# vadimkantorov/convasr

Measured on AMD Instinct MI355X. Metric: audio-seconds/sec/node (fwd+bwd+CTC) at bs64x15s, higher is better.
Workload: dtype bf16

## Files before the change

convasr_amd/_lib.py:

```python
import ctypes
import os

import torch

_HERE = os.path.dirname(os.path.abspath(__file__))
LIB_PATH = os.environ.get('CONVASR_HIP_LIB') or os.path.join(_HERE, 'libconvasr_hip.so')

F32, BF16, I16, F16 = 0, 1, 2, 3
LOSS_SCALER_FLOATS = 8
ACT_NONE, ACT_RELU, ACT_HARDTANH, ACT_LEAKY_RELU = 0, 1, 2, 3
PACK_FWD, PACK_DGRAD = 0, 1
W_REFERENCE, W_KMAJOR = 0, 1
METRIC_CHARS, METRIC_WORDS = 0, 1
METRIC_MAX_LEN = 16383

c_int, c_i64, c_u64, c_f32, c_p = ctypes.c_int, ctypes.c_int64, ctypes.c_uint64, ctypes.c_float, ctypes.c_void_p

_SIGNATURES = dict(
	convasr_abi_version = (c_int, []),
	convasr_last_error = (ctypes.c_char_p, []),
	convasr_convert_layout = (c_int, [c_p, c_int, c_i64, c_i64, c_i64, c_p, c_int, c_i64, c_i64, c_i64, c_int, c_int, c_int, c_p]),
	convasr_signal_absmax = (c_int, [c_p, c_int, c_int, c_int, c_p, c_p]),
	convasr_logmel_fwd = (c_int, [c_p, c_int, c_p, c_p, c_p, c_int, c_p, c_p, c_p, c_int, c_int, c_int, c_int, c_int, c_f32, c_p]),
	convasr_instnorm_fwd = (c_int, [c_p, c_int, c_i64, c_i64, c_i64, c_p, c_int, c_i64, c_i64, c_i64, c_p, c_int, c_int, c_int, c_int, c_f32, c_p]),
	convasr_instnorm_running_fwd = (c_int, [c_p, c_int, c_i64, c_i64, c_i64, c_p, c_int, c_i64, c_i64, c_i64, c_int, c_int, c_int, c_int, c_f32, c_p, c_p, c_p, c_f32, c_int, c_p, c_p]),
	convasr_output_lengths = (c_int, [c_p, c_int, c_int, c_p, c_p]),
	convasr_conv_cout_pad = (c_int, [c_int]),
	convasr_pack_conv_weight = (c_int, [c_p, c_p, c_p, c_int, c_int, c_int, c_int, c_int, c_p]),
	convasr_fold2_geometry = (c_int, [c_int, c_int, ctypes.POINTER(c_int), ctypes.POINTER(c_int)]),
	convasr_fold2_pack_weight = (c_int, [c_p, c_int, c_p, c_int, c_int, c_int, c_int, c_int, c_p]),
	convasr_fold2_unfold_wgrad = (c_int, [c_p, c_p, c_int, c_int, c_int, c_int, c_int, c_int, c_p]),
	convasr_conv1d_fwd = (c_int, [c_p, c_p, c_p, c_int, c_int, c_int, c_int, c_int, c_int, c_int, c_int, c_int, c_int, c_int, c_p, c_p, c_p, c_p, c_int, c_f32, c_f32, c_p, c_p, c_p]),
	convasr_conv_stats_max_rows = (c_int, [c_int, c_int]),
	convasr_grouped_conv1d_fwd = (c_int, [c_p, c_p, c_i64, c_i64, c_i64, c_p, c_p, c_int, c_int, c_int, c_int, c_int, c_int, c_int, c_int, c_int, c_int, c_int, c_p]),
	convasr_grouped_conv1d_dgrad = (c_int, [c_p, c_p, c_p, c_i64, c_i64, c_i64, c_p, c_int, c_int, c_int, c_int, c_int, c_int, c_int, c_int, c_int, c_int, c_p]),
	convasr_grouped_conv1d_wgrad_workspace_bytes = (c_i64, [c_int, c_int, c_int, c_int, c_int]),
	convasr_grouped_conv1d_wgrad = (c_int, [c_p, c_p, c_p, c_p, c_i64, c_i64, c_i64, c_p, c_p, c_int, c_int, c_int, c_int, c_int, c_int, c_int, c_int, c_int, c_int, c_int, c_p]),
	convasr_reduce_rows = (c_int, [c_p, c_int, c_int, c_p, c_p]),
	convasr_debug_set_conv_v2 = (c_int, [c_int]),
	convasr_conv1d_wgrad_workspace_bytes = (c_i64, [c_int, c_int, c_int, c_int, c_int, c_int, c_int, c_int]),
	convasr_conv1d_wgrad = (c_int, [c_p, c_p, c_p, c_p, c_p, c_int, c_int, c_int, c_int, c_int, c_int, c_int, c_int, c_int, c_int, c_int, c_int, c_p]),
	convasr_bn_finalize = (c_int, [c_p, c_int, c_i64, c_p, c_p, c_p, c_p, c_f32, c_f32, c_p, c_p, c_p, c_p, c_int, c_p, c_p]),
	convasr_bn_eval_scale_shift = (c_int, [c_p, c_p, c_p, c_p, c_f32, c_p, c_p, c_int, c_p]),
	convasr_bn_act_fwd = (c_int, [c_p, c_p, c_int, c_p, c_p, c_int, c_p, c_p, c_p, c_int, c_f32, c_f32, c_f32, c_u64, c_u64, c_p, c_p, c_int, c_int, c_int, c_p, c_p]),
	convasr_bn_bwd_workspace_bytes = (c_i64, [c_int, c_int, c_int]),
	convasr_bn_act_bwd_reduce = (c_int, [c_p, c_p, c_p, c_int, c_p, c_p, c_p, c_p, c_int, c_p, c_p, c_p, c_p, c_p, c_p, c_int, c_f32, c_f32, c_f32, c_u64, c_u64, c_p, c_p, c_p, c_p, c_p, c_p, c_p, c_p, c_int, c_int, c_int, c_int, c_p, c_p]),
	convasr_bn_act_bwd_apply = (c_int, [c_p, c_p, c_p, c_int, c_p, c_int, c_p, c_p, c_int, c_f32, c_f32, c_f32, c_u64, c_u64, c_p, c_p, c_int, c_int, c_int, c_p, c_p]),
	convasr_bn_bwd_apply = (c_int, [c_p, c_p, c_p, c_int, c_p, c_p, c_p, c_p, c_p, c_p, c_int, c_int, c_int, c_int, c_p]),
	convasr_log_softmax_fwd = (c_int, [c_p, c_p, c_i64, c_int, c_p]),
	convasr_log_softmax_bwd = (c_int, [c_p, c_p, c_p, c_i64, c_int, c_p]),
	convasr_ctc_workspace_bytes = (c_i64, [c_int, c_int, c_int]),
	convasr_ctc_loss = (c_int, [c_p, c_p, c_p, c_p, c_p, c_p, c_p, c_int, c_int, c_int, c_int, c_int, c_p]),
	convasr_ctc_loss_supported = (c_int, [c_int, c_int, c_int, c_int]),
	convasr_ctc_loss_long_states_per_block = (c_int, []),
	convasr_ctc_loss_long_chunk_frames = (c_int, []),
	convasr_ctc_loss_long_workspace_bytes = (c_i64, [c_int, c_int, c_int, c_int]),
	convasr_ctc_loss_long = (c_int, [c_p, c_p, c_p, c_p, c_p, c_p, c_p, c_i64, c_int, c_int, c_int, c_int, c_int, c_int, c_p]),
	convasr_scale_rows = (c_int, [c_p, c_p, c_p, c_i64, c_p, c_int, c_i64, c_p]),
	convasr_loss_head = (c_int, [c_p, c_p, c_i64, c_p, c_int, c_f32, c_p, c_p, c_p, c_p, c_f32, c_p]),
	convasr_entropy = (c_int, [c_p, c_p, c_p, c_int, c_int, c_int, c_f32, c_p]),
	convasr_weighted_mean_entropy = (c_int, [c_p, c_p, c_p, c_int, c_int, c_int, c_int, c_f32, c_p]),
	convasr_argmax = (c_int, [c_p, c_p, c_i64, c_int, c_p]),
	convasr_sumsq_workspace_bytes = (c_i64, []),
	convasr_sumsq = (c_int, [c_p, c_i64, c_p, c_p, c_p, c_f32, c_p, c_p]),
	convasr_sgd_step = (c_int, [c_p, c_p, c_p, c_p, c_i64, c_p, c_f32, c_f32, c_f32, c_f32, c_int, c_int, c_p, c_f32, c_p, c_int, c_p, c_p, c_p, c_p]),
	convasr_adamw_step = (c_int, [c_p, c_p, c_p, c_p, c_i64, c_p, c_f32, c_f32, c_f32, c_f32, c_f32, c_f32, c_p, c_p, c_p, c_f32, c_p, c_int, c_p, c_p, c_p, c_p]),
	convasr_conv1d_dgrad_bn_reduce = (c_int, [c_p, c_p, c_p, c_int, c_int, c_int, c_int, c_int, c_int, c_int, c_int, c_int, c_p, c_p, c_p, c_p, c_p, c_int, c_f32, c_f32, c_f32, c_u64, c_u64, c_p, c_p, c_p, c_p, c_p, c_p]),
	convasr_bn_bwd_finalize = (c_int, [c_p, c_int, c_p, c_p, c_p, c_p, c_p, c_p, c_int, c_i64, c_int, c_p]),
	convasr_novograd_step = (c_int, [c_p, c_p, c_p, c_p, c_p, c_p, c_p, c_int, c_i64, c_p, c_int, c_p, c_p, c_f32, c_f32, c_f32, c_f32, c_f32, c_f32, c_int, c_int, c_p, c_p, c_f32, c_p, c_int, c_p, c_p, c_p, c_p]),
	convasr_step_begin = (c_int, [c_p, c_p]),
	convasr_conv1x1_grouped = (c_int, [c_int, c_p, c_p, c_p, c_p, c_p, c_p, c_p, c_p, c_int, c_int, c_int, ctypes.POINTER(c_int), c_p]),
	convasr_add16 = (c_int, [c_p, c_p, c_p, c_i64, c_int, c_p]),
	convasr_bn_bwd_reduce_many_workspace_bytes = (c_i64, [c_int, c_int, c_int, c_int]),
	convasr_bn_bwd_reduce_many = (c_int, [c_p, c_p, c_f32, c_p, c_int, c_p, c_p, c_p, c_p, c_p, c_p, c_p, c_p, c_p, c_int, c_int, c_int, c_int, c_p]),
	convasr_pack_dgrad_item_bytes = (c_int, []),
	convasr_pack_dgrad_grouped = (c_int, [c_p, c_int, c_int, c_p]),
	convasr_bn_finalize_grouped = (c_int, [c_int, c_p, c_int, c_i64, c_p, c_p, c_p, c_p, c_p, c_p, c_p, c_p, c_int, c_p]),
	convasr_bn_bwd_finalize_grouped = (c_int, [c_int, c_p, c_p, c_p, c_p, c_p, c_p, c_p, c_p, c_p, c_i64, c_int, c_p]),
	convasr_bn_bwd_apply_grouped = (c_int, [c_p, c_int, c_p, c_p, c_p, c_int, c_int, c_int, c_int, c_p]),
	convasr_wgrad1x1_grouped_workspace_bytes = (c_i64, [c_int, c_p, c_p, c_int, c_int]),
	convasr_wgrad1x1_grouped = (c_int, [c_int, c_p, c_p, c_p, c_p, c_p, c_p, c_p, c_p, c_int, c_int, c_int, c_p]),
	convasr_copy = (c_int, [c_p, c_p, c_i64, c_p]),
	convasr_colsum_workspace_bytes = (c_i64, [c_i64, c_int]),
	convasr_colsum = (c_int, [c_p, c_int, c_i64, c_int, c_p, c_p, c_int, c_p]),
	convasr_cast_scale = (c_int, [c_p, c_int, c_p, c_int, c_i64, c_f32, c_p]),
	convasr_bn_act_fwd_split3 = (c_int, [c_p, c_p, c_int, c_p, c_p, c_int, c_p, c_p, c_p, c_int, c_f32, c_f32, c_f32, c_u64, c_u64, c_p, c_p, c_int, c_int, c_int, c_p, c_p]),
	convasr_bn_act_bwd_apply_split3 = (c_int, [c_p, c_p, c_p, c_int, c_p, c_int, c_p, c_p, c_int, c_f32, c_f32, c_f32, c_u64, c_u64, c_p, c_p, c_int, c_int, c_int, c_p, c_p]),
	convasr_split3 = (c_int, [c_p, c_p, c_int, c_i64, c_int, c_int, c_p]),
	convasr_pack_conv_weight_split3 = (c_int, [c_p, c_int, c_p, c_p, c_int, c_int, c_int, c_int, c_int, c_p]),
	convasr_bn_act_bwd_apply_to_half = (c_int, [c_p, c_p, c_p, c_int, c_p, c_int, c_p, c_p, c_int, c_f32, c_f32, c_f32, c_u64, c_u64, c_p, c_p, c_int, c_int, c_int, c_p, c_p]),
	convasr_conv1d_fwd_splitk_plan = (c_int, [c_int, c_int, c_int, c_int, c_int, c_int, c_p]),
	convasr_conv1d_fwd_splitk = (c_int, [c_p, c_p, c_p, c_int, c_int, c_int, c_int, c_int, c_int, c_int, c_int, c_int, c_int, c_p, c_p, c_p, c_int, c_f32, c_f32, c_p, c_int, c_p, c_p]),
	convasr_conv1d_wgrad_ld_supported = (c_int, [c_int] * 10),
	convasr_conv1d_wgrad_ld = (c_int, [c_p, c_int, c_p, c_int, c_p, c_p, c_int, c_int, c_int, c_int, c_int, c_int, c_int, c_int, c_int, c_int, c_int, c_p]),
	convasr_novograd_item_elems = (c_i64, []),
	convasr_collate_pad = (c_int, [c_p, c_p, c_p, c_p, c_int, c_int, c_int, c_i64, c_p]),
	convasr_ctc_alignment_workspace_bytes = (c_i64, [c_int, c_int, c_int]),
	convasr_ctc_alignment = (c_int, [c_p, c_p, c_p, c_p, c_p, c_p, c_int, c_int, c_int, c_int, c_int, c_p]),
	convasr_ctc_alignment_long_states_per_block = (c_int, []),
	convasr_ctc_alignment_long_chunk_frames = (c_int, []),
	convasr_ctc_alignment_long_workspace_bytes = (c_i64, [c_int, c_int, c_int]),
	convasr_ctc_alignment_long = (c_int, [c_p, c_p, c_p, c_p, c_p, c_p, c_i64, c_int, c_int, c_int, c_int, c_int, c_int, c_p]),
	convasr_ctc_alignment_long_parts = (c_int, [c_p, c_p, c_p, c_p, c_p, c_p, c_i64, c_int, c_int, c_int, c_int, c_int, c_int, c_int, c_p]),
	convasr_ctc_beam_search_workspace_bytes = (c_i64, [c_int] * 6),
	convasr_ctc_beam_search = (c_int, [c_p, c_p, c_p, c_p, c_p, c_p, c_p, c_int, c_int, c_int, c_int, c_int, c_int, c_f32, c_int, c_p]),
	convasr_ctc_beam_search_lm_workspace_bytes = (c_i64, [c_int] * 6),
	convasr_ctc_beam_search_lm = (c_int, [c_p, c_p, c_p, c_p, c_p, c_p, c_p, c_int, c_int, c_int, c_int, c_int, c_int, c_f32, c_int,
	                                      c_p, c_p, c_p, c_int, c_p, c_p, c_int, c_p, c_int, c_int, c_int, c_int, ctypes.c_double, ctypes.c_double, c_p]),
	convasr_ctc_beam_search_wide_workspace_bytes = (c_i64, [c_int] * 6),
	convasr_ctc_beam_search_wide = (c_int, [c_p, c_p, c_p, c_p, c_p, c_p, c_p, c_int, c_int, c_int, c_int, c_int, c_int, c_f32, c_int, c_p]),
	convasr_ctc_beam_search_lm_wide_workspace_bytes = (c_i64, [c_int] * 6),
	convasr_ctc_beam_search_lm_wide = (c_int, [c_p, c_p, c_p, c_p, c_p, c_p, c_p, c_int, c_int, c_int, c_int, c_int, c_int, c_f32, c_int,
	                                           c_p, c_p, c_p, c_int, c_p, c_p, c_int, c_p, c_int, c_int, c_int, c_int, ctypes.c_double, ctypes.c_double, c_p]),
	convasr_edit_distance = (c_int, [c_p, c_p, c_p, c_i64, c_p, c_i64, c_p, c_p, c_int, c_int, c_int, c_int, c_int, c_i64, c_p]),
	convasr_ctc_greedy_collapse = (c_int, [c_p, c_p, c_p, c_p, c_int, c_int, c_int, c_int, c_int, c_p]),
	convasr_ctc_greedy_segments_chunk_frames = (c_int, []),
	convasr_ctc_greedy_segments_workspace_bytes = (c_i64, [c_int, c_int]),
	convasr_ctc_greedy_segments = (c_int, [c_p, c_p, c_p, c_p, c_p, c_p, c_p, c_p, c_p, c_i64, c_int, c_int, c_int, c_int, c_int, c_int, c_p]),
	convasr_nw_align_workspace_bytes = (c_i64, [c_int, c_int, c_int]),
	convasr_nw_align = (c_int, [c_p, c_p, c_p, c_p, c_p, c_p, c_p, c_p, c_p, c_i64, c_int, c_int, c_int, c_int, c_int, c_int, c_int, c_p]),
	convasr_nw_align_long_tile = (c_int, []),
	convasr_nw_align_long_workspace_bytes = (c_i64, [c_int, c_int, c_int]),
	convasr_nw_align_long = (c_int, [c_p, c_p, c_p, c_p, c_p, c_p, c_p, c_p, c_p, c_i64, c_int, c_int, c_int, c_int, c_int, c_int, c_int, c_p]),
	convasr_nw_align_long_parts = (c_int, [c_p, c_p, c_p, c_p, c_p, c_p, c_p, c_p, c_p, c_i64, c_int, c_int, c_int, c_int, c_int, c_int, c_int, c_int, c_p]),
	convasr_edit_distance_long_workspace_bytes = (c_i64, [c_int, c_int, c_int]),
	convasr_edit_distance_long = (c_int, [c_p, c_p, c_p, c_p, c_p, c_p, c_i64, c_int, c_int, c_int, c_p]),
	convasr_sliding_max_out_len = (c_i64, [c_i64, c_int]),
	convasr_sliding_max_tile = (c_int, [c_int]),
	convasr_sliding_max = (c_int, [c_p, c_p, c_int, c_i64, c_int, c_int, c_p]),
	convasr_kth_value_workspace_bytes = (c_i64, [c_int]),
	convasr_kth_value = (c_int, [c_p, c_p, c_p, c_i64, c_int, c_i64, c_i64, c_p]),
	convasr_scan_tile = (c_int, []),
	convasr_sign_prefix_sum_workspace_bytes = (c_i64, [c_i64]),
	convasr_sign_prefix_sum = (c_int, [c_p, c_p, c_p, c_i64, c_i64, c_p]),
	convasr_select_speaker_out_len = (c_i64, [c_i64, c_int, c_int, c_int]),
	convasr_select_speaker_workspace_bytes = (c_i64, [c_i64, c_int, c_int, c_int]),
	convasr_select_speaker = (c_int, [c_p, c_p, c_p, c_p, c_i64, c_i64, c_int, c_int, c_int, c_f32, c_f32, c_f32, c_i64, c_p]),
	convasr_rle1d_workspace_bytes = (c_i64, [c_i64]),
	convasr_rle1d_count_offset = (c_i64, [c_i64]),
	convasr_rle1d_count = (c_int, [c_p, c_int, c_int, c_i64, c_p, c_i64, c_p]),
	convasr_rle1d_write = (c_int, [c_p, c_int, c_int, c_i64, c_p, c_i64, c_i64, c_p, c_p, c_p, c_p]),
	convasr_speaker_error_counts_workspace_bytes = (c_i64, [c_i64]),
	convasr_speaker_error_counts = (c_int, [c_p, c_p, ctypes.POINTER(ctypes.c_int32), c_int, c_i64, c_p, c_p, c_i64, c_p]),
	convasr_resample_tile = (c_int, []),
	convasr_resample_out_len = (c_i64, [c_i64, c_int, c_int]),
	convasr_resample_taps = (c_int, [c_int, c_int, ctypes.c_double, ctypes.c_double]),
	convasr_resample = (c_int, [c_p, c_int, c_i64, c_int, c_int, c_p, c_int, c_int, c_int, c_p, c_i64, c_int, c_p]),
)
SLIDE_ABS, SLIDE_NEG = 1, 2
DIAR_MAX_LEN, DIAR_MAX_KERNEL, RLE_MAX_LEN, SPEAKER_MAX_PERMS = 1 << 28, 16384, 1 << 30, 8

_lib = None


class ConvasrHipError(RuntimeError):
	pass


def declared_symbols():
	return sorted(_SIGNATURES)


def load():
	global _lib
	if _lib is None:
		if not os.path.exists(LIB_PATH):
			raise ConvasrHipError(f'{LIB_PATH} not found: build it with `python -m convasr_amd.build` (hipcc --offload-arch=gfx950)')
		lib = ctypes.CDLL(LIB_PATH)
		if hasattr(lib, 'convasr_debug_read_stamps'):
			lib.convasr_debug_read_stamps.restype, lib.convasr_debug_read_stamps.argtypes = c_int, [c_p, c_int]
			lib.convasr_debug_read_wgrad_stamps.restype, lib.convasr_debug_read_wgrad_stamps.argtypes = c_int, [c_p, c_int]
		for name, (res, args) in _SIGNATURES.items():
			fn = getattr(lib, name)
			fn.restype, fn.argtypes = res, args
		if lib.convasr_abi_version() != 10:
			raise ConvasrHipError('ABI version mismatch')
		_lib = lib
	return _lib


_fns = {}
calls = [0]


def call(name, *args):
	fn = _fns.get(name)
	if fn is None:
		fn = _fns[name] = getattr(load(), name)
	calls[0] += 1
	rc = fn(*args)
	if rc != 0:
		raise ConvasrHipError(f'{name} failed ({rc}): {load().convasr_last_error().decode()}')


def call_rc(name, *args):
	lib = load()
	calls[0] += 1
	rc = getattr(lib, name)(*args)
	if rc < 0:
		raise ConvasrHipError(f'{name} failed ({rc}): {lib.convasr_last_error().decode()}')
	return rc


class _TimingEvent:
	_hip = None
# ... 134 lines not shown
```

convasr_amd/csrc/common.h:

```cpp
#pragma once
#include <hip/hip_runtime.h>
#include <stdint.h>
#include <stdio.h>
#include <stdarg.h>
#include <stdlib.h>
#include "../../include/convasr_hip.h"

typedef unsigned short bf16_t;
typedef _Float16 f16_t;

extern thread_local char g_convasr_err[512];
int convasr_fail(int code, const char* fmt, ...);

#define CONVASR_CHECK_ARG(cond, ...) do { if (!(cond)) return convasr_fail(CONVASR_EINVAL, __VA_ARGS__); } while (0)
#define CONVASR_CHECK_LAUNCH(name) do { hipError_t e_ = hipGetLastError(); if (e_ != hipSuccess) return convasr_fail(CONVASR_ELAUNCH, "%s: %s", name, hipGetErrorString(e_)); } while (0)

static inline int64_t ceil_div64(int64_t a, int64_t b) { return (a + b - 1) / b; }

static inline void convasr_allow_160k_lds(const void* kern, unsigned long long& mask) {
	int dev = 0;
	(void)hipGetDevice(&dev);
	const unsigned long long bit = 1ull << (dev & 63);
	if (!(mask & bit)) { (void)hipFuncSetAttribute(kern, hipFuncAttributeMaxDynamicSharedMemorySize, 160 * 1024); mask |= bit; }
}

static inline int convasr_cu_count() {
	static int cached[64] = {};
	int dev = 0;
	(void)hipGetDevice(&dev);
	int& n = cached[dev & 63];
	if (!n && (hipDeviceGetAttribute(&n, hipDeviceAttributeMultiprocessorCount, dev) != hipSuccess || n <= 0)) n = 256;
	return n;
}

__device__ __forceinline__ float bf16_to_f32(bf16_t v) { return __uint_as_float(((unsigned)v) << 16); }
__device__ __forceinline__ bf16_t f32_to_bf16(float f) {
	__bf16 h = (__bf16)f;
	return __builtin_bit_cast(unsigned short, h);
}

template <typename T> struct Elem;
template <> struct Elem<float> {
	static constexpr int dtype = CONVASR_F32;
	__device__ static __forceinline__ float load(const float* p) { return *p; }
	__device__ static __forceinline__ void store(float* p, float v) { *p = v; }
};
template <> struct Elem<bf16_t> {
	static constexpr int dtype = CONVASR_BF16;
	__device__ static __forceinline__ float load(const bf16_t* p) { return bf16_to_f32(*p); }
	__device__ static __forceinline__ void store(bf16_t* p, float v) { *p = f32_to_bf16(v); }
};

template <> struct Elem<f16_t> {
	static constexpr int dtype = CONVASR_F16;
	__device__ static __forceinline__ float load(const f16_t* p) { return (float)*p; }
	__device__ static __forceinline__ void store(f16_t* p, float v) { *p = (f16_t)v; }
};

template <typename T> __device__ __forceinline__ void unpack16(const uint4& raw, float (&v)[8]);
template <> __device__ __forceinline__ void unpack16<bf16_t>(const uint4& raw, float (&v)[8]) {
	const unsigned w[4] = {raw.x, raw.y, raw.z, raw.w};
#pragma unroll
	for (int i = 0; i < 4; ++i) { v[2 * i] = __uint_as_float(w[i] << 16); v[2 * i + 1] = __uint_as_float(w[i] & 0xffff0000u); }
}
typedef _Float16 f16x2 __attribute__((ext_vector_type(2)));
template <> __device__ __forceinline__ void unpack16<f16_t>(const uint4& raw, float (&v)[8]) {
	const unsigned w[4] = {raw.x, raw.y, raw.z, raw.w};
#pragma unroll
	for (int i = 0; i < 4; ++i) { const f16x2 h = __builtin_bit_cast(f16x2, w[i]); v[2 * i] = (float)h[0]; v[2 * i + 1] = (float)h[1]; }
}
template <typename T> __device__ __forceinline__ unsigned pack16(float lo, float hi);
template <> __device__ __forceinline__ unsigned pack16<bf16_t>(float lo, float hi) { return (unsigned)f32_to_bf16(lo) | ((unsigned)f32_to_bf16(hi) << 16); }
template <> __device__ __forceinline__ unsigned pack16<f16_t>(float lo, float hi) { f16x2 h; h[0] = (f16_t)lo; h[1] = (f16_t)hi; return __builtin_bit_cast(unsigned, h); }

template <typename T> __device__ __forceinline__ void load8(const T* p, float (&v)[8]);
template <> __device__ __forceinline__ void load8<float>(const float* p, float (&v)[8]) {
	float4 a = *reinterpret_cast<const float4*>(p), b = *reinterpret_cast<const float4*>(p + 4);
	v[0] = a.x; v[1] = a.y; v[2] = a.z; v[3] = a.w; v[4] = b.x; v[5] = b.y; v[6] = b.z; v[7] = b.w;
}
template <> __device__ __forceinline__ void load8<bf16_t>(const bf16_t* p, float (&v)[8]) { unpack16<bf16_t>(*reinterpret_cast<const uint4*>(p), v); }
template <> __device__ __forceinline__ void load8<f16_t>(const f16_t* p, float (&v)[8]) { unpack16<f16_t>(*reinterpret_cast<const uint4*>(p), v); }
template <typename T> __device__ __forceinline__ void store8(T* p, const float (&v)[8]);
template <> __device__ __forceinline__ void store8<float>(float* p, const float (&v)[8]) {
	*reinterpret_cast<float4*>(p) = make_float4(v[0], v[1], v[2], v[3]);
	*reinterpret_cast<float4*>(p + 4) = make_float4(v[4], v[5], v[6], v[7]);
}
template <> __device__ __forceinline__ void store8<bf16_t>(bf16_t* p, const float (&v)[8]) {
	*reinterpret_cast<uint4*>(p) = make_uint4(pack16<bf16_t>(v[0], v[1]), pack16<bf16_t>(v[2], v[3]), pack16<bf16_t>(v[4], v[5]), pack16<bf16_t>(v[6], v[7]));
}
template <> __device__ __forceinline__ void store8<f16_t>(f16_t* p, const float (&v)[8]) {
	*reinterpret_cast<uint4*>(p) = make_uint4(pack16<f16_t>(v[0], v[1]), pack16<f16_t>(v[2], v[3]), pack16<f16_t>(v[4], v[5]), pack16<f16_t>(v[6], v[7]));
}

template <typename H> __device__ __forceinline__ void split3_store8(H* out, int C, int order, const float (&v)[8]) {
	float hi[8], lo[8];
	const uint4 ph = make_uint4(pack16<H>(v[0], v[1]), pack16<H>(v[2], v[3]), pack16<H>(v[4], v[5]), pack16<H>(v[6], v[7]));
	unpack16<H>(ph, hi);
#pragma unroll
	for (int k = 0; k < 8; ++k) lo[k] = v[k] - hi[k];
	const uint4 pl = make_uint4(pack16<H>(lo[0], lo[1]), pack16<H>(lo[2], lo[3]), pack16<H>(lo[4], lo[5]), pack16<H>(lo[6], lo[7]));
	*reinterpret_cast<uint4*>(out) = ph;
	*reinterpret_cast<uint4*>(out + C) = order == 0 ? pl : ph;
	*reinterpret_cast<uint4*>(out + 2 * C) = order == 0 ? ph : pl;
}

#define CONVASR_DISPATCH_HALF(dtype, T, ...) do { if ((dtype) == CONVASR_F16) { typedef f16_t T; __VA_ARGS__; } else { typedef bf16_t T; __VA_ARGS__; } } while (0)
static inline bool convasr_is_half(int dtype) { return dtype == CONVASR_BF16 || dtype == CONVASR_F16; }

__device__ __forceinline__ float wave_sum(float v) {
#pragma unroll
	for (int o = 32; o > 0; o >>= 1) v += __shfl_xor(v, o, 64);
	return v;
}
__device__ __forceinline__ float wave_max(float v) {
#pragma unroll
	for (int o = 32; o > 0; o >>= 1) v = fmaxf(v, __shfl_xor(v, o, 64));
	return v;
}

enum { LS_SCALE = 0, LS_UNSKIPPED = 1, LS_OVERFLOW = 2, LS_WINDOW = 3, LS_MIN = 4, LS_MAX = 5, LS_FACTOR = 6, LS_SKIPPED_STEPS = 7 };
struct LossScale { float scale, inv; bool overflow; };
__device__ __forceinline__ LossScale loss_scale_read(const float* __restrict__ scaler, double norm_sq) {
	LossScale r; r.scale = 1.f; r.inv = 1.f; r.overflow = false;
	if (scaler) {
		r.scale = scaler[LS_SCALE];
		r.inv = 1.f / r.scale;
		r.overflow = scaler[LS_WINDOW] > 0.f && !(fabs(norm_sq) < (double)INFINITY);
	}
	return r;
}
__device__ __forceinline__ void loss_scale_advance(const float* __restrict__ in, float* __restrict__ out, bool overflow, bool gated) {
#pragma unroll
	for (int i = 0; i < CONVASR_LOSS_SCALER_FLOATS; ++i) out[i] = in[i];
	if (gated) return;
	float scale = in[LS_SCALE], unskipped = in[LS_UNSKIPPED];
	const float window = in[LS_WINDOW], factor = in[LS_FACTOR];
	out[LS_OVERFLOW] = overflow ? 1.f : 0.f;
	if (window <= 0.f) return;
	if (overflow) { scale = fmaxf(in[LS_MIN], scale / factor); unskipped = 0.f; out[LS_SKIPPED_STEPS] = in[LS_SKIPPED_STEPS] + 1.f; }
	else unskipped += 1.f;
	if (unskipped >= window) { scale = fminf(in[LS_MAX], scale * factor); unskipped = 0.f; }
	out[LS_SCALE] = scale;
	out[LS_UNSKIPPED] = unskipped;
}

__device__ __forceinline__ int valid_len(const float* xlen, int b, int T) {
	if (xlen == nullptr) return T;
	float v = ceilf(xlen[b] * (float)T);
	return (int)v;
}

struct ActConst { float lo, hi, slope, gelse, glo, ghi; int leaky; };
__host__ __device__ __forceinline__ ActConst act_const(int act, float lo, float hi) {
	ActConst c;
	c.lo = -INFINITY; c.hi = INFINITY; c.slope = 1.f; c.gelse = 1.f; c.leaky = 0; c.glo = c.ghi = __builtin_nanf("");
	if (act == CONVASR_ACT_RELU) { c.lo = c.glo = 0.f; c.gelse = 0.f; }
	else if (act == CONVASR_ACT_HARDTANH) { c.lo = c.glo = lo; c.hi = c.ghi = hi; c.gelse = 0.f; }
	else if (act == CONVASR_ACT_LEAKY_RELU) { c.lo = c.glo = 0.f; c.slope = lo; c.gelse = lo; c.leaky = 1; }
	return c;
}
__device__ __forceinline__ float apply_act(float v, const ActConst& c) {
	const float clamped = fminf(fmaxf(v, c.lo), c.hi), lk = v > 0.f ? v : v * c.slope;
	return (c.leaky || v != v) ? lk : clamped;
}
__device__ __forceinline__ float apply_clamp(float v, const ActConst& c) { return v != v ? v : __builtin_amdgcn_fmed3f(v, c.lo, c.hi); }
__device__ __forceinline__ bool act_passes(float pre, const ActConst& c) { return !(pre <= c.glo) && !(pre >= c.ghi); }
__device__ __forceinline__ float act_grad(float pre, const ActConst& c) { return act_passes(pre, c) ? 1.f : c.gelse; }

template <int ROUNDS> __device__ __forceinline__ void philox4x32(uint64_t seed, uint64_t ctr, unsigned (&r)[4]) {
	unsigned c0 = (unsigned)ctr, c1 = (unsigned)(ctr >> 32), c2 = 0, c3 = 0;
	unsigned k0 = (unsigned)seed, k1 = (unsigned)(seed >> 32);
#pragma unroll
	for (int i = 0; i < ROUNDS; ++i) {
		unsigned hi0 = __umulhi(0xD2511F53u, c0), lo0 = 0xD2511F53u * c0;
		unsigned hi1 = __umulhi(0xCD9E8D57u, c2), lo1 = 0xCD9E8D57u * c2;
		unsigned n0 = hi1 ^ c1 ^ k0, n1 = lo1, n2 = hi0 ^ c3 ^ k1, n3 = lo0;
		c0 = n0; c1 = n1; c2 = n2; c3 = n3;
		k0 += 0x9E3779B9u; k1 += 0xBB67AE85u;
	}
	r[0] = c0; r[1] = c1; r[2] = c2; r[3] = c3;
}

__device__ __forceinline__ unsigned lowbias32(unsigned x) {
	x ^= x >> 16; x *= 0x7feb352du;
	x ^= x >> 15; x *= 0x846ca68bu;
	x ^= x >> 16;
	return x;
}

__device__ __forceinline__ unsigned xorshift32(unsigned x) { x ^= x << 13; x ^= x >> 17; x ^= x << 5; return x; }
__device__ __forceinline__ unsigned lowbias32_keyed(unsigned x, unsigned key) {
	x ^= x >> 16; x *= 0x7feb352du;
	x ^= key;
	x ^= x >> 15; x *= 0x846ca68bu;
	x ^= x >> 16;
	return x;
}
__host__ __device__ static inline uint64_t convasr_mix_seed(uint64_t z) {
	z += 0x9E3779B97F4A7C15ull;
	z = (z ^ (z >> 30)) * 0xBF58476D1CE4E5B9ull;
	z = (z ^ (z >> 27)) * 0x94D049BB133111EBull;
	return z ^ (z >> 31);
}

__device__ __forceinline__ void dropout_mask8(uint64_t seed, uint64_t offset, unsigned thr, float scale, int64_t idx, float (&keep)[8]) {
	unsigned r[4];
#ifdef CONVASR_DROPOUT_PHILOX
	philox4x32<7>(seed, offset + (uint64_t)(idx >> 3), r);
#else
	const uint64_t c4 = (offset + (uint64_t)(idx >> 3)) << 2;
	const unsigned key = (unsigned)seed ^ lowbias32((unsigned)(c4 >> 32) ^ (unsigned)(seed >> 32));
	r[0] = lowbias32_keyed((unsigned)c4, key);
#pragma unroll
	for (int i = 1; i < 4; ++i) r[i] = xorshift32(r[i - 1]);
#endif
#pragma unroll
	for (int i = 0; i < 4; ++i) {
		keep[2 * i] = (r[i] & 0xffffu) >= thr ? scale : 0.f;
		keep[2 * i + 1] = (r[i] >> 16) >= thr ? scale : 0.f;
	}
}

__device__ __forceinline__ void philox4(uint64_t seed, uint64_t ctr, float (&u)[4]) {
	unsigned r[4];
	philox4x32<10>(seed, ctr, r);
#pragma unroll
	for (int i = 0; i < 4; ++i) u[i] = (r[i] >> 8) * (1.0f / 16777216.0f);
}
```

convasr_amd/csrc/ctc.hip:

```cpp
#include "common.h"

#define CTC_NEG (-1e30f)
#define CTC_DEAD (-1e29f)
#define CTC_LOG2E 1.4426950408889634f
#define CTC_LN2 0.6931471805599453
#define CTC_RENORM 8
#define CTC_RENORM_LOG2 3
#define CTC_EMPTY 0xFFFFFFFFu
#ifndef CTC_SPIN_LIMIT
#define CTC_SPIN_LIMIT (1 << 22)
#endif

__device__ __forceinline__ float lse3(float a, float b, float c) {
	const float m = fmaxf(a, fmaxf(b, c));
	const float md = __builtin_amdgcn_fmed3f(a, b, c), lo = fminf(a, fminf(b, c));
	return m + __builtin_amdgcn_logf(1.f + __builtin_amdgcn_exp2f(md - m) + __builtin_amdgcn_exp2f(lo - m));
}
__device__ __forceinline__ float lse2(float a, float b) {
	const float m = __builtin_amdgcn_fmed3f(a, b, INFINITY);
	return m + __builtin_amdgcn_logf(1.f + __builtin_amdgcn_exp2f(__builtin_amdgcn_fmed3f(a, b, -INFINITY) - m));
}

__device__ __forceinline__ float wave_shr1(float v, float fill) {
	return __builtin_bit_cast(float, __builtin_amdgcn_update_dpp(__builtin_bit_cast(int, fill), __builtin_bit_cast(int, v), 0x138, 0xf, 0xf, false));
// ... 74 lines not shown
		if (t == CONVASR_CTC_SKIP_PUBLISH) return;
#endif
		if (!consumes && edge_lane) {
			if (FWD) slot_store(q.edge + t, ctc_word(a[NS - 1]));
			else { slot_store(q.edge + 2 * t, ctc_word(a[0])); slot_store(q.edge + 2 * t + 1, ctc_word(a[1])); }
		}
	};
	{
		const float* row = q.lpb + (int64_t)t0 * CS;
#pragma unroll
		for (int i = 0; i < NS; ++i) {
			const int s = s0 + i;
			a[i] = ((FWD ? s < 2 : s >= L - 2) && valid[i]) ? score(row[cls[i]], i) : CTC_NEG;
		}
		store_states<NS>(lat + (int64_t)t0 * LP, a);
		if (lane == 0) { q.off[0] = 0.f; if (!consumes) slot_store(q.ecum, ctc_word(0.f)); }
		publish(t0);
		if (Tb > 1) {
#pragma unroll
			for (int i = 0; i < NS; ++i) cur[i] = score(q.lpb[(int64_t)(t0 + dt) * CS + cls[i]], i);
		}
	}
	uint32_t x0 = CTC_EMPTY, x1 = FWD ? 0u : CTC_EMPTY, xc = 0;
	for (int k = 1; k < Tb; ++k) {
		const int t = t0 + k * dt;
		float e0 = CTC_NEG, e1 = CTC_NEG;
		if (consumes) {
			const uint32_t* e = q.edge + (int64_t)(t - dt) * EW;
			if (__builtin_expect(x0 == CTC_EMPTY || x1 == CTC_EMPTY, 0)) {
				int spins = 0;
				do {
					x0 = slot_load(e);
					if (!FWD) x1 = slot_load(e + 1);
				} while ((x0 == CTC_EMPTY || x1 == CTC_EMPTY) && ++spins < CTC_SPIN_LIMIT);
				if (spins >= CTC_SPIN_LIMIT) *q.gave_up = 1.f;
				xc = slot_load(q.ecum + ((k - 1) >> CTC_RENORM_LOG2));
			}
			const float d = __builtin_bit_cast(float, xc) - cum;
			e0 = __builtin_bit_cast(float, x0) + d;
			if (!FWD) e1 = __builtin_bit_cast(float, x1) + d;
			x0 = slot_load(e + dt * EW);
			if (!FWD) x1 = slot_load(e + dt * EW + 1);
			xc = slot_load(q.ecum + (k >> CTC_RENORM_LOG2));
		}
		if (k + 1 < Tb) {
#pragma unroll
			for (int i = 0; i < NS; ++i) nxt[i] = q.lpb[(int64_t)(t + dt) * CS + cls[i]];
		}
		float n[NS];
		if (FWD) {
			float p1 = wave_shr1(a[NS - 1], CTC_NEG);
			if (lane == 0) p1 = e0;
#pragma unroll
			for (int i = NS - 1; i >= 0; --i) {
				const float m1 = i >= 1 ? a[i >= 1 ? i - 1 : 0] : p1;
				const float m2 = i >= 2 ? a[i >= 2 ? i - 2 : 0] : p1;
				n[i] = ((i & 1) ? lse3(a[i], m1, skip[i] ? m2 : CTC_NEG) : lse2(a[i], m1)) + cur[i];
			}
		} else {
			float q0 = wave_shl1(a[0], CTC_NEG), q1 = wave_shl1(a[1], CTC_NEG);
			if (lane == 63) { q0 = e0; q1 = e1; }
#pragma unroll
			for (int i = 0; i < NS; ++i) {
				const float m1 = i + 1 < NS ? a[i + 1 < NS ? i + 1 : 0] : q0;
				const float m2 = i + 2 < NS ? a[i + 2 < NS ? i + 2 : 0] : q1;
				n[i] = ((i & 1) ? lse3(a[i], m1, skip[i] ? m2 : CTC_NEG) : lse2(a[i], m1)) + cur[i];
			}
		}
		if ((k & (CTC_RENORM - 1)) == 0) {
			float m = n[0];
#pragma unroll
			for (int i = 1; i < NS; ++i) m = fmaxf(m, n[i]);
			m = wave_max_dpp(m);
			if (m > CTC_DEAD && m < INFINITY) {
				const float kk = floorf(m);
#pragma unroll
				for (int i = 0; i < NS; ++i) n[i] -= kk;
				cum += kk;
			}
			if (lane == 0) { q.off[k >> CTC_RENORM_LOG2] = cum; if (!consumes) slot_store(q.ecum + (k >> CTC_RENORM_LOG2), ctc_word(cum)); }
		}
#pragma unroll
		for (int i = 0; i < NS; ++i) a[i] = n[i];
		store_states<NS>(lat + (int64_t)t * LP, a);
		publish(t);
#pragma unroll
		for (int i = 0; i < NS; ++i) cur[i] = score(nxt[i], i);
	}
	if (FWD) {
#pragma unroll
		for (int i = 0; i < NS; ++i) q.fin[s0 + i] = a[i];
		if (lane == 0) q.fcum[0] = cum;
	}
}

template <int NPH, int NPL, bool LP_LDS>
__global__ __launch_bounds__(256) void ctc_alpha_beta_kernel(const float* __restrict__ lp, const int64_t* __restrict__ targets, const int64_t* __restrict__ olen,
                                                             const int64_t* __restrict__ ylen, float* __restrict__ nll, float* __restrict__ alpha,
                                                             float* __restrict__ beta, float* __restrict__ offs, float* __restrict__ tot,
                                                             int B, int T, int C, int S_max, int blank) {
	extern __shared__ __attribute__((aligned(16))) float ctc_smem[];
	constexpr int CAP = 128 * (NPH + NPL);
	const int NB = T / CTC_RENORM + 1;
	float* const fin = ctc_smem;
	float* const fcum = fin + CAP;
	uint32_t* const edge = reinterpret_cast<uint32_t*>(fcum + 4);
	const int n_edge = 3 * T + 2 * NB;
	float* const lpl = fcum + 4 + ((n_edge + 3) & ~3);
	const int b = blockIdx.x;
	const int Tb = (int)olen[b], S = (int)ylen[b], L = 2 * S + 1;
	const float* lpg = lp + (int64_t)b * T * C;
	if (Tb <= 0 || Tb > T) {
		if (threadIdx.x == 0) nll[b] = (Tb == 0 && S == 0) ? 0.f : INFINITY;
		return;
	}
	for (int i = threadIdx.x; i < n_edge; i += blockDim.x) edge[i] = CTC_EMPTY;
	if (threadIdx.x == 0) fcum[2] = 0.f;
	if (LP_LDS) {
		const int n = Tb * (C + 1);
		for (int i = threadIdx.x; i < n; i += blockDim.x) {
			const int t = i / (C + 1), c = i - t * (C + 1);
			lpl[i] = c < C ? ctc_floor(lpg[(int64_t)t * C + c] * CTC_LOG2E) : CTC_NEG;
		}
	}
	__syncthreads();
	const int wave = __builtin_amdgcn_readfirstlane(threadIdx.x >> 6);
	const bool fwd = wave < 2;
	CtcSweep q;
	q.lpb = LP_LDS ? lpl : lpg;
	q.tg = targets + (int64_t)b * S_max;
	q.lat = (fwd ? alpha : beta) + (int64_t)b * T * CAP;
	q.off = offs + (((int64_t)(fwd ? 0 : 1) * B + b) * 2 + (wave & 1)) * NB;
	q.edge = edge + (fwd ? 0 : T);
	q.ecum = edge + 3 * T + (fwd ? 0 : NB);
	q.fin = fin; q.fcum = fcum + (wave & 1); q.gave_up = fcum + 2;
	q.T = T; q.C = C; q.Tb = Tb; q.L = L; q.blank = blank; q.cap = CAP; q.lane = threadIdx.x & 63;
	q.s_base = wave == 1 ? 128 * NPH : (wave == 3 ? 128 * NPL : 0);
	if (wave == 0) ctc_sweep<NPH, true, false, LP_LDS>(q);
	else if (wave == 1) ctc_sweep<NPL, true, true, LP_LDS>(q);
	else if (wave == 2) ctc_sweep<NPL, false, true, LP_LDS>(q);
	else ctc_sweep<NPH, false, false, LP_LDS>(q);
	__syncthreads();
	if (threadIdx.x == 0) {
		const float c1 = fcum[L - 1 >= 128 * NPH];
		const float l1 = fin[L - 1], l2 = L >= 2 ? fin[L - 2] + (fcum[L - 2 >= 128 * NPH] - c1) : CTC_NEG;
		const float m = fmaxf(l1, l2);
		const float rem = m + log2f(exp2f(l1 - m) + exp2f(l2 - m));
		nll[b] = fcum[2] != 0.f ? NAN : (m > CTC_DEAD ? (float)(-CTC_LN2 * ((double)c1 + (double)rem)) : INFINITY);
		tot[2 * b] = c1;
		tot[2 * b + 1] = rem;
	}
}

__global__ __launch_bounds__(256) void ctc_grad_kernel(const float* __restrict__ lp, const int64_t* __restrict__ targets, const int64_t* __restrict__ olen,
                                                       const int64_t* __restrict__ ylen, const float* __restrict__ nll, const float* __restrict__ alpha,
                                                       const float* __restrict__ beta, const float* __restrict__ offs, const float* __restrict__ tot, float* __restrict__ grad,
                                                       int B, int T, int C, int S_max, int blank, int t_per_block, int cap, int split_a, int split_b) {
	extern __shared__ float bins[];
	const int NB = T / CTC_RENORM + 1;
	const int b = blockIdx.y, lane = threadIdx.x & 63, wave = threadIdx.x >> 6;
	const int Tb = (int)olen[b], S = (int)ylen[b], L = 2 * S + 1;
	const bool feasible = nll[b] < INFINITY;
	const int64_t* tg = targets + (int64_t)b * S_max;
	float* mybins = bins + wave * C;
	const int t_begin = blockIdx.x * t_per_block, t_end = min(T, t_begin + t_per_block);
	for (int t = t_begin + wave; t < t_end; t += 4) {
		const float* row = lp + ((int64_t)b * T + t) * C;
		float* grow = grad + ((int64_t)b * T + t) * C;
		if (t >= Tb || !feasible) {
			for (int c = lane; c < C; c += 64) grow[c] = 0.f;
			continue;
		}
		for (int c = lane; c < C; c += 64) mybins[c] = 0.f;
		__builtin_amdgcn_s_waitcnt(0xc07f);
		__builtin_amdgcn_wave_barrier();
		const float* ar = alpha + ((int64_t)b * T + t) * cap;
		const float* br = beta + ((int64_t)b * T + t) * cap;
		const float* oa = offs + (int64_t)b * 2 * NB + (t >> CTC_RENORM_LOG2);
		const float* ob = offs + ((int64_t)B + b) * 2 * NB + ((Tb - 1 - t) >> CTC_RENORM_LOG2);
		const float ti = tot[2 * b], tr = tot[2 * b + 1];
		const float oa0 = oa[0] - ti, oa1 = oa[NB] - ti, ob0 = ob[0], ob1 = ob[NB];
		const float lpb = row[blank] * CTC_LOG2E;
		float blank_sum = 0.f;
		for (int s = lane; s < L; s += 64) {
			const float shift = ((s >= split_a ? oa1 : oa0) + (s >= split_b ? ob1 : ob0)) - tr;
			const float ab = ar[s] + br[s];
			if (s & 1) {
				const int c = (int)tg[s >> 1];
				atomicAdd(mybins + c, __builtin_amdgcn_exp2f(ab + (shift - row[c] * CTC_LOG2E)));
			} else blank_sum += __builtin_amdgcn_exp2f(ab + (shift - lpb));
		}
		blank_sum = wave_sum(blank_sum);
		if (lane == 0) atomicAdd(mybins + blank, blank_sum);
		__builtin_amdgcn_s_waitcnt(0xc07f);
		__builtin_amdgcn_wave_barrier();
		for (int c = lane; c < C; c += 64) grow[c] = __expf(row[c]) - mybins[c];
		__builtin_amdgcn_wave_barrier();
	}
}

static int ctc_split(int S_max, int* nph, int* npl) {
	const int pairs = (2 * S_max + 1 + 127) / 128;
	if (pairs > 16) return -1;
	const int p = pairs < 2 ? 2 : pairs;
	*nph = (p + 1) / 2;
	*npl = p / 2;
	return 0;
}

extern "C" int64_t convasr_ctc_workspace_bytes(int B, int T, int S_max) {
	int nph, npl;
	if (ctc_split(S_max, &nph, &npl) < 0) return -1;
	const int NB = T / CTC_RENORM + 1;
	return (2 * (int64_t)B * T * 128 * (nph + npl) + 4 * (int64_t)B * NB + 2 * (int64_t)B) * (int64_t)sizeof(float);
}

static size_t ctc_lds_fixed(int T, int cap) {
	const int64_t NB = T / CTC_RENORM + 1;
	return (size_t)(cap + 4 + ((3 * (int64_t)T + 2 * NB + 3) & ~(int64_t)3)) * sizeof(float);
}

extern "C" int convasr_ctc_loss_supported(int B, int T, int C, int S_max) {
	int nph, npl;
	if (B <= 0 || T <= 0 || C <= 1 || C > 8192 || S_max < 0 || ctc_split(S_max, &nph, &npl) < 0) return 0;
	return ctc_lds_fixed(T, 128 * (nph + npl)) <= 159 * 1024 ? 1 : 0;
}

extern "C" int convasr_ctc_loss(const float* log_probs, const int64_t* targets, const int64_t* olen, const int64_t* ylen, float* nll, float* grad,
                                void* workspace, int B, int T, int C, int S_max, int blank, void* stream) {
	CONVASR_CHECK_ARG(log_probs && targets && olen && ylen && nll && workspace && B > 0 && T > 0 && C > 1 && S_max >= 0 && blank >= 0 && blank < C, "ctc_loss: bad arguments");
	int nph, npl;
	if (ctc_split(S_max, &nph, &npl) < 0) return convasr_fail(CONVASR_EUNSUPPORTED, "ctc_loss: target length %d > 1023", S_max);
	CONVASR_CHECK_ARG(C <= 8192, "ctc_loss: C %d > 8192", C);
	hipStream_t s = (hipStream_t)stream;
	const int NB = T / CTC_RENORM + 1, cap = 128 * (nph + npl);
	float* alpha = (float*)workspace;
	float* beta = alpha + (int64_t)B * T * cap;
	float* offs = beta + (int64_t)B * T * cap;
	float* tot = offs + 4 * (int64_t)B * NB;
	const int t_per_block = 32;
	dim3 ggrid((T + t_per_block - 1) / t_per_block, B);
	const size_t gsmem = 4 * (size_t)C * sizeof(float);
	const size_t lds_fixed = ctc_lds_fixed(T, cap), lds_lp = (size_t)T * (C + 1) * sizeof(float);
	CONVASR_CHECK_ARG(lds_fixed <= 159 * 1024, "ctc_loss: T %d too long for the edge slots", T);
	const bool in_lds = lds_fixed + lds_lp <= 159 * 1024;
#define CTC_LAUNCH(NPH, NPL, LDS) do { \
		auto kern = ctc_alpha_beta_kernel<NPH, NPL, LDS>; \
		static unsigned long long set = 0; \
		convasr_allow_160k_lds(reinterpret_cast<const void*>(kern), set); \
		hipLaunchKernelGGL(kern, dim3(B), dim3(256), lds_fixed + (LDS ? lds_lp : 0), s, log_probs, targets, olen, ylen, nll, alpha, beta, offs, tot, B, T, C, S_max, blank); \
	} while (0)
#define CTC_CASE(NPH, NPL) case NPH + NPL: if (in_lds) CTC_LAUNCH(NPH, NPL, true); else CTC_LAUNCH(NPH, NPL, false); break;
	switch (nph + npl) {
		CTC_CASE(1, 1) CTC_CASE(2, 1) CTC_CASE(2, 2) CTC_CASE(3, 2) CTC_CASE(3, 3) CTC_CASE(4, 3) CTC_CASE(4, 4)
		CTC_CASE(5, 4) CTC_CASE(5, 5) CTC_CASE(6, 5) CTC_CASE(6, 6) CTC_CASE(7, 6) CTC_CASE(7, 7) CTC_CASE(8, 7) CTC_CASE(8, 8)
	}
#undef CTC_CASE
#undef CTC_LAUNCH
	if (grad) hipLaunchKernelGGL(ctc_grad_kernel, ggrid, dim3(256), gsmem, s, log_probs, targets, olen, ylen, nll, alpha, beta, offs, tot, grad, B, T, C, S_max, blank, t_per_block, cap, 128 * nph, 128 * npl);
	CONVASR_CHECK_LAUNCH("ctc_loss");
	return 0;
}
```

convasr_amd/csrc/misc.hip:

```cpp
#include "common.h"

thread_local char g_convasr_err[512] = {0};

int convasr_fail(int code, const char* fmt, ...) {
	va_list ap;
	va_start(ap, fmt);
	vsnprintf(g_convasr_err, sizeof(g_convasr_err), fmt, ap);
	va_end(ap);
	return code;
}

extern "C" int convasr_abi_version(void) { return CONVASR_ABI_VERSION; }
extern "C" const char* convasr_last_error(void) { return g_convasr_err; }

template <typename S, typename D>
__global__ __launch_bounds__(256) void convert_layout_kernel(const S* __restrict__ src, int64_t ssb, int64_t ssc, int64_t sst,
                                                             D* __restrict__ dst, int64_t dsb, int64_t dsc, int64_t dst_st, int C, int T) {
	__shared__ float tile[64][65];
	const int b = blockIdx.z, c0 = blockIdx.y * 64, t0 = blockIdx.x * 64;
	const int tx = threadIdx.x & 63, ty = threadIdx.x >> 6;
	const bool src_t_fast = (sst == 1) || (ssc != 1), dst_t_fast = (dst_st == 1) || (dsc != 1);
#pragma unroll 4
	for (int i = 0; i < 16; ++i) {
		int c = src_t_fast ? c0 + ty + 4 * i : c0 + tx, t = src_t_fast ? t0 + tx : t0 + ty + 4 * i;
// ... 2 lines not shown
		tile[c - c0][t - t0] = v;
	}
	__syncthreads();
#pragma unroll 4
	for (int i = 0; i < 16; ++i) {
		int c = dst_t_fast ? c0 + ty + 4 * i : c0 + tx, t = dst_t_fast ? t0 + tx : t0 + ty + 4 * i;
		if (c < C && t < T) Elem<D>::store(dst + b * dsb + c * dsc + t * dst_st, tile[c - c0][t - t0]);
	}
}

extern "C" int convasr_convert_layout(const void* src, int src_dtype, int64_t ssb, int64_t ssc, int64_t sst, void* dst, int dst_dtype,
                                      int64_t dsb, int64_t dsc, int64_t dst_st, int B, int C, int T, void* stream) {
	CONVASR_CHECK_ARG(src && dst && B > 0 && C > 0 && T > 0, "convert_layout: bad arguments");
	dim3 grid((T + 63) / 64, (C + 63) / 64, B);
	hipStream_t s = (hipStream_t)stream;
#define LAUNCH(S, D) hipLaunchKernelGGL((convert_layout_kernel<S, D>), grid, dim3(256), 0, s, (const S*)src, ssb, ssc, sst, (D*)dst, dsb, dsc, dst_st, C, T)
	if (src_dtype == CONVASR_F32 && dst_dtype == CONVASR_F32) LAUNCH(float, float);
	else if (src_dtype == CONVASR_F32 && dst_dtype == CONVASR_BF16) LAUNCH(float, bf16_t);
	else if (src_dtype == CONVASR_BF16 && dst_dtype == CONVASR_F32) LAUNCH(bf16_t, float);
	else if (src_dtype == CONVASR_BF16 && dst_dtype == CONVASR_BF16) LAUNCH(bf16_t, bf16_t);
	else if (src_dtype == CONVASR_F32 && dst_dtype == CONVASR_F16) LAUNCH(float, f16_t);
	else if (src_dtype == CONVASR_F16 && dst_dtype == CONVASR_F32) LAUNCH(f16_t, float);
	else if (src_dtype == CONVASR_F16 && dst_dtype == CONVASR_F16) LAUNCH(f16_t, f16_t);
	else return convasr_fail(CONVASR_EUNSUPPORTED, "convert_layout: dtype %d -> %d", src_dtype, dst_dtype);
#undef LAUNCH
	CONVASR_CHECK_LAUNCH("convert_layout");
	return 0;
}

template <typename S, typename D>
__global__ __launch_bounds__(1024) void instnorm_kernel(const S* __restrict__ x, int64_t xsb, int64_t xsc, int64_t xst, D* __restrict__ y,
                                                        int64_t ysb, int64_t ysc, int64_t yst, const float* __restrict__ xlen, int C, int T, int T_out, float eps,
                                                        float* __restrict__ stats_out, const float* __restrict__ fixed_mean, const float* __restrict__ fixed_var) {
	__shared__ float red[64][17];
	__shared__ float bc[16];
	const int b = blockIdx.y, cl = threadIdx.x & 15, c = blockIdx.x * 16 + cl, tl = threadIdx.x >> 4;
	const int n = valid_len(xlen, b, T);
	const bool ok = c < C;
	const S* xp = x + b * xsb + (ok ? c : 0) * xsc;
	auto block_sum = [&](float v) {
		red[tl][cl] = v;
		__syncthreads();
		if (threadIdx.x < 16) { float s = 0.f; for (int i = 0; i < 64; ++i) s += red[i][threadIdx.x]; bc[threadIdx.x] = s; }
		__syncthreads();
		return bc[cl];
	};
	float mean, stdv;
	if (fixed_mean) {
		mean = ok ? fixed_mean[c] : 0.f;
		stdv = sqrtf((ok ? fixed_var[c] : 1.f) + eps);
	} else {
		float acc = 0.f;
		for (int t = tl; t < n; t += 64) acc += ok ? Elem<S>::load(xp + t * xst) : 0.f;
		mean = block_sum(acc) / (float)n;
		acc = 0.f;
		for (int t = tl; t < n; t += 64) { float d = ok ? Elem<S>::load(xp + t * xst) - mean : 0.f; acc += d * d; }
		const float var = block_sum(acc) / (float)n;
		stdv = sqrtf(var + eps);
		if (stats_out && ok && tl == 0) { stats_out[((int64_t)b * C + c) * 2] = mean; stats_out[((int64_t)b * C + c) * 2 + 1] = var; }
	}
	if (!ok) return;
	D* yp = y + b * ysb + c * ysc;
	for (int t = tl; t < T_out; t += 64) {
		float v = t < n ? (Elem<S>::load(xp + t * xst) - mean) / stdv : 0.f;
		Elem<D>::store(yp + t * yst, v);
	}
}

static int instnorm_launch(const void* x, int x_dtype, int64_t xsb, int64_t xsc, int64_t xst, void* y, int y_dtype, int64_t ysb, int64_t ysc, int64_t yst, const float* xlen,
                           int B, int C, int T, int T_out, float eps, float* stats_out, const float* fixed_mean, const float* fixed_var, hipStream_t s);

extern "C" int convasr_instnorm_fwd(const void* x, int x_dtype, int64_t xsb, int64_t xsc, int64_t xst, void* y, int y_dtype, int64_t ysb,
                                    int64_t ysc, int64_t yst, const float* xlen, int B, int C, int T, int T_out, float eps, void* stream) {
	CONVASR_CHECK_ARG(x && y && B > 0 && C > 0 && T > 0 && T_out >= T, "instnorm_fwd: bad arguments");
	hipStream_t s = (hipStream_t)stream;
	return instnorm_launch(x, x_dtype, xsb, xsc, xst, y, y_dtype, ysb, ysc, yst, xlen, B, C, T, T_out, eps, nullptr, nullptr, nullptr, s);
}

static int instnorm_launch(const void* x, int x_dtype, int64_t xsb, int64_t xsc, int64_t xst, void* y, int y_dtype, int64_t ysb, int64_t ysc, int64_t yst, const float* xlen,
                           int B, int C, int T, int T_out, float eps, float* stats_out, const float* fixed_mean, const float* fixed_var, hipStream_t s) {
	dim3 grid((C + 15) / 16, B);
#define LAUNCH(S, D) hipLaunchKernelGGL((instnorm_kernel<S, D>), grid, dim3(1024), 0, s, (const S*)x, xsb, xsc, xst, (D*)y, ysb, ysc, yst, xlen, C, T, T_out, eps, stats_out, fixed_mean, fixed_var)
	if (x_dtype == CONVASR_F32 && y_dtype == CONVASR_F32) LAUNCH(float, float);
	else if (x_dtype == CONVASR_F32 && y_dtype == CONVASR_BF16) LAUNCH(float, bf16_t);
	else if (x_dtype == CONVASR_BF16 && y_dtype == CONVASR_F32) LAUNCH(bf16_t, float);
	else if (x_dtype == CONVASR_BF16 && y_dtype == CONVASR_BF16) LAUNCH(bf16_t, bf16_t);
	else if (x_dtype == CONVASR_F32 && y_dtype == CONVASR_F16) LAUNCH(float, f16_t);
	else if (x_dtype == CONVASR_F16 && y_dtype == CONVASR_F32) LAUNCH(f16_t, float);
	else if (x_dtype == CONVASR_F16 && y_dtype == CONVASR_F16) LAUNCH(f16_t, f16_t);
	else return convasr_fail(CONVASR_EUNSUPPORTED, "instnorm_fwd: dtype %d -> %d", x_dtype, y_dtype);
#undef LAUNCH
	CONVASR_CHECK_LAUNCH("instnorm_fwd");
	return 0;
}

__global__ void instnorm_running_kernel(const float* __restrict__ stats, int B, int C, int T, float momentum, float* __restrict__ rmean, float* __restrict__ rvar, long long* __restrict__ nbt) {
	const int c = blockIdx.x * blockDim.x + threadIdx.x;
	if (c == 0 && nbt) *nbt += 1;
	if (c >= C) return;
	float m = 0.f, v = 0.f;
	const float unbias = T > 1 ? (float)T / (float)(T - 1) : 1.f;
	for (int b = 0; b < B; ++b) { m += stats[((int64_t)b * C + c) * 2]; v += stats[((int64_t)b * C + c) * 2 + 1] * unbias; }
	rmean[c] = (1.f - momentum) * rmean[c] + momentum * (m / (float)B);
	rvar[c] = (1.f - momentum) * rvar[c] + momentum * (v / (float)B);
}

extern "C" int convasr_instnorm_running_fwd(const void* x, int x_dtype, int64_t xsb, int64_t xsc, int64_t xst, void* y, int y_dtype, int64_t ysb, int64_t ysc, int64_t yst,
                                            int B, int C, int T, int T_out, float eps, float* running_mean, float* running_var, int64_t* num_batches_tracked, float momentum,
                                            int training, float* stats_workspace, void* stream) {
	CONVASR_CHECK_ARG(x && y && running_mean && running_var && B > 0 && C > 0 && T > 0 && T_out >= T && (!training || stats_workspace), "instnorm_running_fwd: bad arguments");
	hipStream_t s = (hipStream_t)stream;
	if (!training) return instnorm_launch(x, x_dtype, xsb, xsc, xst, y, y_dtype, ysb, ysc, yst, nullptr, B, C, T, T_out, eps, nullptr, running_mean, running_var, s);
	const int rc = instnorm_launch(x, x_dtype, xsb, xsc, xst, y, y_dtype, ysb, ysc, yst, nullptr, B, C, T, T_out, eps, stats_workspace, nullptr, nullptr, s);
	if (rc) return rc;
	hipLaunchKernelGGL(instnorm_running_kernel, dim3((C + 63) / 64), dim3(64), 0, s, (const float*)stats_workspace, B, C, T, momentum, running_mean, running_var, (long long*)num_batches_tracked);
	CONVASR_CHECK_LAUNCH("instnorm_running_fwd");
	return 0;
}

__global__ void output_lengths_kernel(const float* __restrict__ xlen, int B, int T, int64_t* __restrict__ out) {
	const int b = blockIdx.x * blockDim.x + threadIdx.x;
	if (b < B) out[b] = (int64_t)valid_len(xlen, b, T);
}

extern "C" int convasr_output_lengths(const float* xlen, int B, int T, int64_t* out, void* stream) {
	CONVASR_CHECK_ARG(out && B > 0 && T >= 0, "output_lengths: bad arguments");
	hipLaunchKernelGGL(output_lengths_kernel, dim3((B + 255) / 256), dim3(256), 0, (hipStream_t)stream, xlen, B, T, out);
	CONVASR_CHECK_LAUNCH("output_lengths");
	return 0;
}

__global__ __launch_bounds__(256) void log_softmax_fwd_kernel(const float* __restrict__ x, float* __restrict__ y, int64_t rows, int C) {
	const int64_t row = (int64_t)blockIdx.x * 4 + (threadIdx.x >> 6);
	const int lane = threadIdx.x & 63;
	if (row >= rows) return;
	const float* xp = x + row * C;
	float m = -INFINITY;
	for (int c = lane; c < C; c += 64) m = fmaxf(m, xp[c]);
	m = wave_max(m);
	float s = 0.f;
	for (int c = lane; c < C; c += 64) s += expf(xp[c] - m);
	s = wave_sum(s);
	const float lse = m + logf(s);
	for (int c = lane; c < C; c += 64) y[row * C + c] = xp[c] - lse;
}

__global__ __launch_bounds__(256) void log_softmax_bwd_kernel(const float* __restrict__ g, const float* __restrict__ lp, float* __restrict__ dx, int64_t rows, int C) {
	const int64_t row = (int64_t)blockIdx.x * 4 + (threadIdx.x >> 6);
	const int lane = threadIdx.x & 63;
	if (row >= rows) return;
	float s = 0.f;
	for (int c = lane; c < C; c += 64) s += g[row * C + c];
	s = wave_sum(s);
	for (int c = lane; c < C; c += 64) dx[row * C + c] = g[row * C + c] - expf(lp[row * C + c]) * s;
}

extern "C" int convasr_log_softmax_fwd(const float* logits, float* log_probs, int64_t rows, int C, void* stream) {
	CONVASR_CHECK_ARG(logits && log_probs && rows > 0 && C > 0, "log_softmax_fwd: bad arguments");
	hipLaunchKernelGGL(log_softmax_fwd_kernel, dim3((unsigned)ceil_div64(rows, 4)), dim3(256), 0, (hipStream_t)stream, logits, log_probs, rows, C);
	CONVASR_CHECK_LAUNCH("log_softmax_fwd");
	return 0;
}

extern "C" int convasr_log_softmax_bwd(const float* grad_lp, const float* log_probs, float* dlogits, int64_t rows, int C, void* stream) {
	CONVASR_CHECK_ARG(grad_lp && log_probs && dlogits && rows > 0 && C > 0, "log_softmax_bwd: bad arguments");
	hipLaunchKernelGGL(log_softmax_bwd_kernel, dim3((unsigned)ceil_div64(rows, 4)), dim3(256), 0, (hipStream_t)stream, grad_lp, log_probs, dlogits, rows, C);
	CONVASR_CHECK_LAUNCH("log_softmax_bwd");
	return 0;
}

__global__ __launch_bounds__(1024) void entropy_kernel(const float* __restrict__ lp, const int64_t* __restrict__ olen, float* __restrict__ ent, int T, int C, float eps) {
	__shared__ float red[16];
	const int b = blockIdx.x, w = threadIdx.x >> 6, lane = threadIdx.x & 63;
	const int n = olen ? (int)olen[b] : T;
	const int total = min(n, T) * C;
	const float* p = lp + (int64_t)b * T * C;
	float a0 = 0.f, a1 = 0.f;
	int i = threadIdx.x;
	for (; i + 1024 < total; i += 2048) { const float v0 = p[i], v1 = p[i + 1024]; a0 -= expf(v0) * v0; a1 -= expf(v1) * v1; }
	if (i < total) { const float v = p[i]; a0 -= expf(v) * v; }
	float acc = wave_sum(a0 + a1);
	if (lane == 0) red[w] = acc;
	__syncthreads();
	if (threadIdx.x == 0) {
		float s = 0.f;
		for (int k = 0; k < 16; ++k) s += red[k];
		ent[b] = olen ? s / (eps + (float)n) : s / (float)T;
	}
}

extern "C" int convasr_entropy(const float* log_probs, const int64_t* olen, float* ent, int B, int T, int C, float eps, void* stream) {
	CONVASR_CHECK_ARG(log_probs && ent && B > 0 && T > 0 && C > 0, "entropy: bad arguments");
	hipLaunchKernelGGL(entropy_kernel, dim3(B), dim3(1024), 0, (hipStream_t)stream, log_probs, olen, ent, T, C, eps);
	CONVASR_CHECK_LAUNCH("entropy");
	return 0;
}

__global__ __launch_bounds__(1024) void weighted_entropy_kernel(const float* __restrict__ lp, const int64_t* __restrict__ olen, float* __restrict__ out, int T, int C, int eps_id, float eps) {
	__shared__ float red[2][16];
	const int b = blockIdx.x, w = threadIdx.x >> 6, lane = threadIdx.x & 63;
	const int n = olen ? min((int)olen[b], T) : T;
	const float* p = lp + (int64_t)b * T * C;
	float num = 0.f, den = 0.f;
	for (int t = w; t < n; t += 16) {
		float e = 0.f, sil = 0.f;
		for (int c = lane; c < C; c += 64) {
			const float v = p[(int64_t)t * C + c], pr = expf(v);
			e -= pr * v;
			if (c == eps_id) sil = pr;
		}
		e = wave_sum(e);
		sil = wave_sum(sil);
		const float wt = 1.f - sil;
		num += e * wt;
		den += wt;
	}
	if (lane == 0) { red[0][w] = num; red[1][w] = den; }
	__syncthreads();
	if (threadIdx.x == 0) {
		float a = 0.f, d = 0.f;
		for (int k = 0; k < 16; ++k) { a += red[0][k]; d += red[1][k]; }
		out[b] = a / (eps + d);
	}
}

extern "C" int convasr_weighted_mean_entropy(const float* log_probs, const int64_t* olen, float* out, int B, int T, int C, int eps_id, float eps, void* stream) {
	CONVASR_CHECK_ARG(log_probs && out && B > 0 && T > 0 && C > 0 && eps_id >= 0 && eps_id < C, "weighted_mean_entropy: bad arguments");
	hipLaunchKernelGGL(weighted_entropy_kernel, dim3(B), dim3(1024), 0, (hipStream_t)stream, log_probs, olen, out, T, C, eps_id, eps);
	CONVASR_CHECK_LAUNCH("weighted_mean_entropy");
	return 0;
}

__device__ __forceinline__ bool argmax_beats(float v, int i, float best, int bi) {
	const bool vn = v != v, bn = best != best;
	if (vn || bn) return vn && (!bn || i < bi);
	return v > best || (v == best && i < bi);
}

__global__ __launch_bounds__(256) void argmax_kernel(const float* __restrict__ lp, int64_t* __restrict__ idx, int64_t rows, int C) {
	const int64_t row = (int64_t)blockIdx.x * 4 + (threadIdx.x >> 6);
	const int lane = threadIdx.x & 63;
	if (row >= rows) return;
	float best = -INFINITY;
	int bi = 0x7fffffff;
	for (int c = lane; c < C; c += 64) { float v = lp[row * C + c]; if (argmax_beats(v, c, best, bi)) { best = v; bi = c; } }
#pragma unroll
	for (int o = 32; o > 0; o >>= 1) {
		float ov = __shfl_xor(best, o, 64);
		int oi = __shfl_xor(bi, o, 64);
		if (argmax_beats(ov, oi, best, bi)) { best = ov; bi = oi; }
	}
	if (lane == 0) idx[row] = bi;
}

extern "C" int convasr_argmax(const float* log_probs, int64_t* idx, int64_t rows, int C, void* stream) {
	CONVASR_CHECK_ARG(log_probs && idx && rows > 0 && C > 0, "argmax: bad arguments");
	hipLaunchKernelGGL(argmax_kernel, dim3((unsigned)ceil_div64(rows, 4)), dim3(256), 0, (hipStream_t)stream, log_probs, idx, rows, C);
	CONVASR_CHECK_LAUNCH("argmax");
	return 0;
}

__global__ __launch_bounds__(256) void scale_rows_kernel(const float* __restrict__ g, const float* __restrict__ sc, const int64_t* __restrict__ div, int64_t div_stride, float* __restrict__ out, int64_t per_b) {
	const int b = blockIdx.y;
	const float s0 = sc ? sc[b] : 1.f;
	const float s = div ? s0 / (float)div[b * div_stride] : s0;
	for (int64_t i = (int64_t)blockIdx.x * 256 + threadIdx.x; i < per_b; i += (int64_t)gridDim.x * 256) out[b * per_b + i] = g[b * per_b + i] * s;
}

extern "C" int convasr_scale_rows(const float* grad, const float* gscale, const int64_t* gdiv, int64_t gdiv_stride, float* out, int B, int64_t per_b, void* stream) {
	CONVASR_CHECK_ARG(grad && (gscale || gdiv) && out && B > 0 && per_b > 0, "scale_rows: bad arguments");
	unsigned gx = (unsigned)(ceil_div64(per_b, 256) > 64 ? 64 : ceil_div64(per_b, 256));
	hipLaunchKernelGGL(scale_rows_kernel, dim3(gx, B), dim3(256), 0, (hipStream_t)stream, grad, gscale, gdiv, gdiv_stride, out, per_b);
	CONVASR_CHECK_LAUNCH("scale_rows");
	return 0;
}

__global__ __launch_bounds__(256) void loss_head_kernel(const float* __restrict__ lv, const int64_t* __restrict__ ylen, int64_t ylen_stride, const float* __restrict__ ent, int B, float accum,
                                                        float* __restrict__ out, float* __restrict__ gvec, unsigned char* __restrict__ skipped, const float* __restrict__ scaler, float metric_scale) {
	__shared__ float red[3][256];
	float a = 0.f, c = 0.f, e = 0.f;
	const float gbase = (1.f / accum) / (float)B, ls = scaler ? scaler[LS_SCALE] : 1.f;
	for (int b = threadIdx.x; b < B; b += 256) {
		const float w = (float)ylen[b * ylen_stride], l = lv[b];
		a += l * w;
		c += l;
		if (ent) e += ent[b];
		if (gvec) gvec[b] = gbase * w * ls;
	}
	red[0][threadIdx.x] = a; red[1][threadIdx.x] = c; red[2][threadIdx.x] = e;
	__syncthreads();
	for (int o = 128; o > 0; o >>= 1) {
		if ((int)threadIdx.x < o) { red[0][threadIdx.x] += red[0][threadIdx.x + o]; red[1][threadIdx.x] += red[1][threadIdx.x + o]; red[2][threadIdx.x] += red[2][threadIdx.x + o]; }
		__syncthreads();
	}
	if (threadIdx.x == 0) {
		const float cur = red[1][0] / (float)B;
		out[0] = red[0][0] / (float)B / accum;
		out[1] = cur * metric_scale;
		out[2] = red[2][0] / (float)B * metric_scale;
		if (skipped) *skipped = (fabsf(cur) < INFINITY) ? 0 : 1;
	}
}

__global__ void step_begin_kernel(uint64_t* __restrict__ st) {
	const uint64_t step = st[1] + 1;
	st[1] = step;
	st[2] = convasr_mix_seed(st[0] ^ convasr_mix_seed(step));
// ... 244 lines not shown
```

convasr_amd/functional.py:

```python
import os

import torch

from . import ops, _lib
from . import weights as W

_PLANES_ATTR = '_convasr_planes_only'
_PLANES_CACHE_ATTR = '_convasr_planes_cache'
_nan_cells = {}


def _planes_placeholder(z3, B, C, T):
	dev = z3.device
	cell = _nan_cells.get(dev)
	if cell is None:
		cell = _nan_cells[dev] = torch.full((1, ), float('nan'), dtype = torch.float32, device = dev)
	z = cell.as_strided((B, C, T), (0, 0, 0))
	setattr(z, _PLANES_ATTR, z3)
	return z


def _take_planes(x):
	d = getattr(x, '__dict__', None)
	return d.pop(_PLANES_ATTR, None) if d else None
# ... 417 lines not shown
			rsum_of = {r: sums[2 * Cout * (1 + i):2 * Cout * (2 + i)] for i, r in enumerate(bn_idx)}
			common = dict(xlen = xl, res = res_y, rscale = [None if p is None else p[2] for p in res_bnp], rshift = [None if p is None else p[3] for p in res_bnp], rmean = [None if p is None else p[0] for p in res_bnp], rinvstd = [None if p is None else p[1] for p in res_bnp], dropout_p = p_drop, seed = seed, offset = offset, step_key = skey)
			first = [r for r in bn_idx if r < 2]
			g = ops.bn_act_bwd_reduce(dz, y, bnp[2], bnp[3], bnp[0], bnp[1], act, rsums = [rsum_of.get(r) if r in first else None for r in range(n_res)], sums = sums[:2 * Cout], **common)
			rest = [r for r in bn_idx if r >= 2]
			while rest:
				batch, rest = rest[:2], rest[2:]
				ops.bn_act_bwd_reduce(g, g, None, None, None, None, (_lib.ACT_NONE, 0.0, 0.0), res = [res_y[r] for r in batch], rscale = [None] * len(batch), rshift = [None] * len(batch), rmean = [common['rmean'][r] for r in batch], rinvstd = [common['rinvstd'][r] for r in batch], rsums = [rsum_of[r] for r in batch], write_g = False)
			grouped_bn = GROUP_RES and dt in ops.HALF_DTYPES and len(bn_idx) >= 1 and len(bn_idx) <= 12
			if grouped_bn:
				coefs = torch.empty(1 + len(bn_idx), 3 * Cout, dtype = torch.float32, device = dev)
				sets = [(gamma, beta, bnp, sums[:2 * Cout])] + [(ctx.params[3 + 4 * r + 2], ctx.params[3 + 4 * r + 3], res_bnp[r], rsum_of[r]) for r in bn_idx]
				dgb = _deliver_many([[gm, bt] for gm, bt, _, _ in sets], lambda outs, accs: ops.bn_bwd_finalize_grouped([t[3] for t in sets], [t[0] for t in sets], [t[2][0] for t in sets], [t[2][1] for t in sets], B * Tout,
					[coefs[i] for i in range(len(sets))], [o[0] for o in outs], [o[1] for o in outs], accs), always = True)
				dys = ops.bn_bwd_apply_grouped(g, [y] + [res_y[r] for r in bn_idx], [coefs[i] for i in range(len(sets))])
				(dgamma, dbeta), dy = dgb[0], dys[0]
				grouped_bn = {r: (dgb[1 + i][0], dgb[1 + i][1], dys[1 + i]) for i, r in enumerate(bn_idx)}
			else:
				dgamma, dbeta, dy = _bn_backward_from_g(g, y, gamma, beta, bnp, sums[:2 * Cout], B * Tout)

		if n_res == 0:
			grouped_bn = None
		arena_mode = getattr(weight, '_convasr_grad', None) is not None
		if ctx.split is not None and dy.dtype == torch.float32:
			dy = ops.as_cl(dy, ctx.split) if hi else ops.split3(dy, ctx.split, ops.SPLIT_GRAD)
		if hi and ctx.fold is not None:
			wg = lambda: _deliver([weight], lambda outs, acc: Fold2.wgrad_hi(x, dy, weight, spec, ctx.fold[0], ctx.fold[1], outs[0], acc))
		elif hi:
			wg = lambda: _deliver([weight], lambda outs, acc: ops.conv1d_wgrad_hi(x, dy, Cout, spec.K, spec.dilation, spec.padding, outs[0], accumulate = acc))
		elif ctx.split is not None and ctx.fold is not None:
			wg = lambda: _deliver([weight], lambda outs, acc: Fold2.wgrad_split(x, dy, weight, spec, ctx.fold[0], ctx.fold[1], outs[0], acc))
		elif ctx.split is not None:
			xf, dyf = ops.split3_frames(x), ops.split3_frames(dy)
			wg = lambda: _deliver([weight], lambda outs, acc: ops.conv1d_wgrad(xf, dyf, Cout, spec.K, 1, 3 * spec.dilation, 3 * spec.padding, outs[0], accumulate = acc, work = 2.0 * B * Tout * Cout * weight.shape[1] * spec.K, family = SPLIT_WGRAD_FAMILY))
		elif ctx.fold is not None:
			Bx, Cin, Tin = x.shape
			xv = x.as_strided((Bx, 2 * Cin, Tin // 2), (Tin * Cin, 1, 2 * Cin))
			wg = lambda: _deliver([weight], lambda outs, acc: Fold2.wgrad(xv, dy, weight, spec, ctx.fold[0], ctx.fold[1], outs[0], acc))
		else:
			wg = lambda: _deliver([weight], lambda outs, acc: ops.conv1d_wgrad(x, dy, Cout, spec.K, spec.stride, spec.dilation, spec.padding, outs[0], accumulate = acc))
		if arena_mode:
			dw, = _run_wgrad(dev, (x, dy), wg)
		dx = None
		if ctx.x_needs_grad:
			if spec.stride != 1:
				raise _lib.ConvasrHipError('conv1d dgrad with stride > 1 is not implemented (only the prologue conv is strided and its input needs no gradient)')
			dx = _dgrad(x, dy, weight, spec, dt, ctx.producer_link, split = ctx.split, hi = hi)
		if not arena_mode:
			dw, = wg()

		res_grads = [None] * (5 * n_res)
		pending = []
		wg_group = []
		for r in range(n_res):
			rw, rb, rg, rbeta = ctx.params[3 + 4 * r:3 + 4 * r + 4]
			rx = res_x[r]
			need_rx = ctx.needs_input_grad[6 + 5 * r]
			if res_bnp[r] is None:
				res_grads[5 * r] = g if need_rx else None
				continue
			p = res_bnp[r]
			drg, drbeta, dry = grouped_bn[r] if grouped_bn else _bn_backward_from_g(g, res_y[r], rg, rbeta, p, rsum_of[r], B * Tout)
			drx = None
			if ctx.res_split[r]:
				sp, cin_r = cfg['split'], rw.shape[1]
				hi_r = bool(cfg.get('split_hi_bwd'))
				dry3 = ops.as_cl(dry, sp) if hi_r else ops.split3(dry, sp, ops.SPLIT_GRAD)
				if need_rx and hi_r:
					drx = ops.conv1d(dry3, W.split_weight(rw, sp, 1)[1], cin_r, 1, 1, 1, 0, out_dtype = torch.float32)
				elif need_rx:
					drx = ops.conv1d(dry3, W.split_weight(rw, sp)[1], cin_r, 1, 1, 1, 0, out_dtype = torch.float32, work = 2.0 * B * Tout * Cout * cin_r, family = SPLIT_FAMILY)

				def res_wgrad3(outs, acc, rx3 = rx, dry3 = dry3, rb = rb, cin_r = cin_r, hi_r = hi_r):
					if hi_r:
						ops.conv1d_wgrad_hi(rx3, dry3, Cout, 1, 1, 0, outs[0], accumulate = acc)
					else:
						ops.conv1d_wgrad(ops.split3_frames(rx3), ops.split3_frames(dry3), Cout, 1, 1, 3, 0, outs[0], accumulate = acc, work = 2.0 * B * Tout * Cout * cin_r, family = SPLIT_WGRAD_FAMILY)
					if outs[1] is not None and not acc and not (outs[1] is getattr(rb, '_convasr_grad', None) and getattr(rb, '_convasr_grad_is_zero', False)):
						outs[1].zero_()
						rb._convasr_grad_is_zero = outs[1] is getattr(rb, '_convasr_grad', None)
				drw, drb = _deliver([rw, rb], res_wgrad3)
				res_grads[5 * r:5 * r + 5] = [drx, drw, drb, drg, drbeta]
				continue
			if need_rx and ctx.res_gacc[r] is not None and rx.shape[1] % 128 == 0 and Cout % 64 == 0:
				pending.append((r, dry))
			elif need_rx:
				W.join_prepack(dry.device)
				drx = ops.conv1d(dry, W.packed_weight(rw, dt, _lib.PACK_DGRAD), rx.shape[1], 1, 1, 1, 0)
			arena = getattr(rw, '_convasr_grad', None) is not None and (rb is None or getattr(rb, '_convasr_grad', None) is not None)
			if GROUP_RES and arena and rw.requires_grad and dt in ops.HALF_DTYPES and rx.shape[1] % 128 == 0 and Cout % 128 == 0 and (rb is None or rb.requires_grad):
				wg_group.append((r, rx, dry))
				res_grads[5 * r:5 * r + 5] = [drx, None, None, drg, drbeta]
				continue
			def res_wgrad(outs, acc, rx = rx, dry = dry, rb = rb):
				ops.conv1d_wgrad(rx, dry, Cout, 1, 1, 1, 0, outs[0], accumulate = acc)
				if outs[1] is not None and not acc and not (outs[1] is getattr(rb, '_convasr_grad', None) and getattr(rb, '_convasr_grad_is_zero', False)):
					outs[1].zero_()
					rb._convasr_grad_is_zero = outs[1] is getattr(rb, '_convasr_grad', None)
			if RES_WGRAD_SIDE and arena:
				drw, drb = _run_wgrad(dry.device, (rx, dry), lambda rw = rw, rb = rb, f = res_wgrad: _deliver([rw, rb], f))
			else:
				drw, drb = _deliver([rw, rb], res_wgrad)
			res_grads[5 * r:5 * r + 5] = [drx, drw, drb, drg, drbeta]
		if pending:
			W.join_prepack(dev)
			accs = [ctx.res_gacc[r] for r, _ in pending]
			fresh = [a['buf'] is None for a in accs]
			for (r, _), a, fr in zip(pending, accs, fresh):
				if fr:
					a['buf'] = ops.empty_cl(B, res_x[r].shape[1], Tout, dt, dev)
			done = ops.conv1x1_grouped([dry for _, dry in pending], [W.packed_weight(ctx.params[3 + 4 * r], dt, _lib.PACK_DGRAD) for r, _ in pending], [res_x[r].shape[1] for r, _ in pending], outs = [a['buf'] for a in accs], accumulate = [not fr for fr in fresh])
			if done is None:
				raise _lib.ConvasrHipError('grouped input gradient of the residual branches: a shape left the one-tap kernel\'s envelope between forward and backward')
		if wg_group:
			ps = [(ctx.params[3 + 4 * r], ctx.params[3 + 4 * r + 1]) for r, _, _ in wg_group]
			fresh = [_arenas_fresh([p_ for p_ in wb if p_ is not None]) for wb in ps]

			def run():
				ok = ops.wgrad1x1_grouped([rx for _, rx, _ in wg_group], [dry for _, _, dry in wg_group], [w._convasr_grad for w, _ in ps], zeros = [b._convasr_grad if (b is not None and fr) else None for (_, b), fr in zip(ps, fresh)], accumulate = [not fr for fr in fresh])
				if not ok:
					raise _lib.ConvasrHipError('grouped weight gradient of the residual branches: a shape outside the kernel\'s envelope')
			if RES_WGRAD_SIDE:
				_run_wgrad(dev, tuple(t for _, rx, dry in wg_group for t in (rx, dry)), run)
			else:
				run()
			filled = [p_ for wb in ps for p_ in wb if p_ is not None]
			for p_ in filled:
				p_._convasr_grad_is_zero = False
			_mark_delivered(filled)
		return (None, dx, dw, dgamma, dbeta, None, *res_grads)


def _momentum(bn):
	if bn.momentum is None:
		if CAPTURING[0]:
			raise _lib.ConvasrHipError('a batch norm with momentum = None (cumulative average: its factor is read from the device every step) cannot be captured into a step graph')
		return 1.0 / float(int(bn.num_batches_tracked.item()) + 1)
	return bn.momentum


def _stats_buffer(bn, C, dev, B, Tout, slot = '_convasr_stats'):
	if CAPTURING[0]:
		return ops.ConvStats(C, B, Tout, dev)
	st = getattr(bn, slot, None)
	if st is None or not st.fits(C, B, Tout, dev):
		st = ops.ConvStats(C, B, Tout, dev)
		setattr(bn, slot, st)
	return st


class _HeadPad:
	_pad_bufs = {}

	@classmethod
	def pad_grad(cls, dy, dt):
		B, Cout, T = dy.shape
		key = (B, T, Cout, dt, dy.device, torch.cuda.current_stream(dy.device).cuda_stream)
		out = None if CAPTURING[0] else cls._pad_bufs.get(key)
		if CAPTURING[0]:
			out = ops.zeros_cl(B, W.HEAD_PAD, T, dt, dy.device)
		elif out is None:
			if len(cls._pad_bufs) >= 64:
				cls._pad_bufs.clear()
			out = cls._pad_bufs[key] = ops.zeros_cl(B, W.HEAD_PAD, T, dt, dy.device)
		_lib.call('convasr_convert_layout', _lib.ptr(dy), _lib.dtype_code(dy.dtype), dy.stride(0), dy.stride(1), dy.stride(2), _lib.ptr(out), _lib.dtype_code(dt), out.stride(0), out.stride(1), out.stride(2), B, Cout, T, _lib.stream_ptr())
		return out


class ConvBiasFunction(torch.autograd.Function):

	@staticmethod
	def forward(ctx, cfg, x, weight, bias):
		spec, dt = cfg['spec'], cfg['compute_dtype']
		ctx.producer_link = _take_link(x)
		x = ops.as_cl(x, dt)
		Cout, Cin, K = weight.shape
		ctx.split = None
		if cfg.get('split') is not None and dt == torch.float32 and K == 1 and spec.stride == 1 and spec.padding == 0 and Cin % 128 == 0 and Cout <= W.HEAD_PAD and os.environ.get('CONVASR_NO_HEAD_PAD') != '1':
			ctx.split = cfg['split']
			B, _, T = x.shape
			x = ops.split3(x, ctx.split, ops.SPLIT_INPUT)
			y = ops.conv1d(x, W.head_split_weight(weight, ctx.split, 1 if cfg.get('split_hi_bwd') else 3)[0], Cout, 1, 1, 1, 0, out_dtype = cfg.get('out_dtype', torch.float32), bias = bias, work = 2.0 * B * T * Cout * Cin, family = SPLIT_FAMILY)
		else:
			y = ops.conv1d(x, W.packed_weight(weight, dt, _lib.PACK_FWD), weight.shape[0], spec.K, spec.stride, spec.dilation, spec.padding, out_dtype = cfg.get('out_dtype', torch.float32), bias = bias)
		ctx.cfg = cfg
		ctx.params = (weight, bias)
		ctx.save_for_backward(x)
		return y

	@staticmethod
	def backward(ctx, dy):
		cfg = ctx.cfg
		spec, dt = cfg['spec'], cfg['compute_dtype']
		weight, bias = ctx.params
		x, = ctx.saved_tensors
		Cout = weight.shape[0]
		if ctx.split is not None:
			Cin = weight.shape[1]
			B, _, T = dy.shape
			dy = ops.as_cl(dy, torch.float32)
			hi = bool(cfg.get('split_hi_bwd'))
			dy3 = _HeadPad.pad_grad(dy, ctx.split) if hi else ops.split3(_HeadPad.pad_grad(dy, torch.float32), ctx.split, ops.SPLIT_GRAD)
			dx = None
			if ctx.needs_input_grad[1] and hi:
				dx = ops.conv1d(dy3, W.head_split_weight(weight, ctx.split, 1)[1], Cin, 1, 1, 1, 0, out_dtype = torch.float32, work = 2.0 * B * T * Cout * Cin)
				_after_long_launch()
			elif ctx.needs_input_grad[1]:
				dx = ops.conv1d(dy3, W.head_split_weight(weight, ctx.split)[1], Cin, 1, 1, 1, 0, out_dtype = torch.float32, work = 2.0 * B * T * Cout * Cin, family = SPLIT_FAMILY)
				_after_long_launch()

			def wgrad3(outs, acc):
				dwp = torch.empty(W.HEAD_PAD, Cin, 1, dtype = torch.float32, device = dy.device)
				if hi:
					ops.conv1d_wgrad_hi(x, dy3, W.HEAD_PAD, 1, 1, 0, dwp, work = 2.0 * B * T * Cout * Cin)
				else:
					ops.conv1d_wgrad(ops.split3_frames(x), ops.split3_frames(dy3), W.HEAD_PAD, 1, 1, 3, 0, dwp, work = 2.0 * B * T * Cout * Cin, family = SPLIT_WGRAD_FAMILY)
				if outs[0] is not None:
					v = dwp[:Cout]
					if acc:
						outs[0].add_(v.view(outs[0].shape))
					else:
						_lib.call('convasr_convert_layout', _lib.ptr(v), _lib.F32, 0, v.stride(0), v.stride(1), _lib.ptr(outs[0]), _lib.F32, 0, outs[0].stride(0), outs[0].stride(1), 1, Cout, Cin, _lib.stream_ptr())
				if outs[1] is not None:
					ops.colsum(dy, outs[1], accumulate = acc)
			dw, db = _deliver([weight, bias], wgrad3)
			return None, dx, dw, db
		if dt in ops.HALF_DTYPES and spec.K == 1 and spec.stride == 1 and spec.padding == 0 and Cout < W.HEAD_PAD and x.shape[1] % 128 == 0 and os.environ.get('CONVASR_NO_HEAD_PAD') != '1':
			dyp = _HeadPad.pad_grad(dy, dt)
			dx = _dgrad(x, dyp, weight, spec, dt, ctx.producer_link, wd = W.head_dgrad_weight(weight, dt)) if ctx.needs_input_grad[1] else None

			def wgrad(outs, acc):
				dwp = torch.empty(W.HEAD_PAD, x.shape[1], 1, dtype = torch.float32, device = x.device)
				dbp = torch.empty(W.HEAD_PAD, dtype = torch.float32, device = x.device) if outs[1] is not None else None
				ops.conv1d_wgrad(x, dyp, W.HEAD_PAD, 1, 1, 1, 0, dwp, dbias = dbp)
				for o, v in ((outs[0], dwp[:Cout]), (outs[1], None if dbp is None else dbp[:Cout].view(Cout, 1, 1))):
					if o is None:
						continue
					if acc:
						o.add_(v.view(o.shape))
					else:
						ov = o.view(Cout, -1, 1) if o.ndim == 1 else o
						_lib.call('convasr_convert_layout', _lib.ptr(v), _lib.F32, 0, v.stride(0), v.stride(1), _lib.ptr(ov), _lib.F32, 0, ov.stride(0), ov.stride(1), 1, Cout, v.shape[1], _lib.stream_ptr())
			dw, db = _deliver([weight, bias], wgrad)
			return None, dx, dw, db
		dy = ops.as_cl(dy, dt)
		dx = None
		if ctx.needs_input_grad[1]:
			if spec.stride != 1:
				raise _lib.ConvasrHipError('conv1d dgrad with stride > 1 is not implemented')
			dx = _dgrad(x, dy, weight, spec, dt, ctx.producer_link)
		dw, db = _deliver([weight, bias], lambda outs, acc: ops.conv1d_wgrad(x, dy, Cout, spec.K, spec.stride, spec.dilation, spec.padding, outs[0], dbias = outs[1], accumulate = acc))
		return None, dx, dw, db


class GroupedConvReluFunction(torch.autograd.Function):

	@staticmethod
	def forward(ctx, cfg, x, weight, bias):
		spec, dt = cfg['spec'], cfg['compute_dtype']
		_take_link(x)
		x = ops.as_cl(x, dt)
		y = ops.grouped_conv1d(x, weight.detach(), None if bias is None else bias.detach(), cfg['groups'], spec.stride, spec.padding, relu = True)
		ctx.cfg, ctx.params = cfg, (weight, bias)
		ctx.save_for_backward(x, y)
		return y

	@staticmethod
	def backward(ctx, dy):
		cfg = ctx.cfg
		spec, dt, groups = cfg['spec'], cfg['compute_dtype'], cfg['groups']
		weight, bias = ctx.params
		x, y = ctx.saved_tensors
		dy = ops.as_cl(dy, dt)
		dx = ops.grouped_conv1d_dgrad(dy, y, weight.detach(), x.shape[1], x.shape[2], groups, spec.stride, spec.padding) if ctx.needs_input_grad[1] else None
		dw, db = _deliver([weight, bias], lambda outs, acc: ops.grouped_conv1d_wgrad(x, dy, y, outs[0], outs[1], groups, spec.stride, spec.padding, accumulate = acc))
		return None, dx, dw, db


class ConvBnActEvalFunction:

	@staticmethod
	def apply(cfg, x, weight, bias, scale_shift, xlen, res_list):
		spec, dt, act = cfg['spec'], cfg['compute_dtype'], cfg['act']
		x = ops.as_cl(x, dt)
		Cout = weight.shape[0]
		xl = ops.xlen_f32(xlen, x.device) if (cfg['temporal_mask'] and xlen is not None) else None
		scale, shift = (None, None) if scale_shift is None else (scale_shift[0], scale_shift[1])
		fold = Fold2.plan(x, weight, spec, dt, False)
		sk = not torch.is_grad_enabled()
		split = cfg.get('split_eval')
		if fold is not None:
			xv, Kf, Pf, Tout = fold
			conv = lambda **epilogue: ops.conv1d(xv, W.fold2_packed_weight(weight, dt, spec.padding), Cout, Kf, 1, 1, Pf, bias = bias, Tout = Tout, work = 2.0 * x.shape[0] * Tout * Cout * x.shape[1] * spec.K, splitk = sk, **epilogue)
		elif split_applies(split, dt, spec, x.shape[1], Cout):
			x3, wp3 = ops.split3(x, split, ops.SPLIT_INPUT), W.split_weight(weight, split)[0]
			conv = lambda **epilogue: ops.conv1d(x3, wp3, Cout, spec.K, 1, spec.dilation, spec.padding, out_dtype = torch.float32, bias = bias, work = 2.0 * x.shape[0] * ops.conv_out_len(x.shape[2], spec.K, 1, spec.dilation, spec.padding) * Cout * x.shape[1] * spec.K, family = SPLIT_FAMILY, splitk = sk, **epilogue)
		else:
			wp = W.packed_weight(weight, dt, _lib.PACK_FWD)
			conv = lambda **epilogue: ops.conv1d(x, wp, Cout, spec.K, spec.stride, spec.dilation, spec.padding, bias = bias, splitk = sk, **epilogue)
		p_drop = float(cfg.get('dropout_p', 0.0))
		if not res_list and p_drop == 0:
			return conv(scale = scale, shift = shift, act = act, xlen = xl)
		y = conv()
		res_y, rscale, rshift = [], [], []
		for rx, rw, rb, rss in res_list:
			rx = ops.as_cl(rx, dt)
			if rw is None:
				res_y.append(rx); rscale.append(None); rshift.append(None)
			elif split_applies(split, dt, ConvSpec(1), rx.shape[1], Cout):
				res_y.append(ops.conv1d(ops.split3(rx, split, ops.SPLIT_INPUT), W.split_weight(rw, split)[0], Cout, 1, 1, 1, 0, out_dtype = torch.float32, bias = rb, work = 2.0 * rx.shape[0] * rx.shape[2] * Cout * rx.shape[1], family = SPLIT_FAMILY, splitk = sk))
				rscale.append(None if rss is None else rss[0]); rshift.append(None if rss is None else rss[1])
			else:
				res_y.append(ops.conv1d(rx, W.packed_weight(rw, dt, _lib.PACK_FWD), Cout, 1, 1, 1, 0, bias = rb, splitk = sk))
				rscale.append(None if rss is None else rss[0]); rshift.append(None if rss is None else rss[1])
		seed, offset = _DropoutState.next(y.numel()) if p_drop > 0 else (0, 0)
		return ops.bn_act(y, scale, shift, act, xlen = xl, res = res_y, rscale = rscale, rshift = rshift, dropout_p = p_drop, seed = seed, offset = offset, step_key = _DropoutState.key(y.device) if p_drop > 0 else None)


class ConvBnActFrozenStatsFunction(torch.autograd.Function):

	@staticmethod
	def _affine(bn, gamma, beta):
		if bn is None or not isinstance(bn, torch.nn.modules.batchnorm._BatchNorm):
			return None, None, None, None
		ss = ops.bn_eval_scale_shift(gamma, beta, bn.running_mean, bn.running_var, bn.eps)
		return ss[0], ss[1], bn.running_mean.detach().float(), torch.rsqrt(bn.running_var.detach().float() + bn.eps)

	@staticmethod
	def forward(ctx, cfg, x, weight, bias, gamma, beta, xlen, *flat_res):
		spec, dt, act = cfg['spec'], cfg['compute_dtype'], cfg['act']
		ctx.producer_link = _take_link(x)
		x = ops.as_cl(x, dt)
		dev = x.device
		Cout = weight.shape[0]
		xl = ops.xlen_f32(xlen, dev) if (cfg['temporal_mask'] and xlen is not None) else None
		y = ops.conv1d(x, W.packed_weight(weight, dt, _lib.PACK_FWD), Cout, spec.K, spec.stride, spec.dilation, spec.padding, bias = bias)
		aff = ConvBnActFrozenStatsFunction._affine(cfg['bn'], gamma, beta)
		n_res = len(flat_res) // 5
		res_x, res_y, res_aff = [], [], []
		for r in range(n_res):
			rx, rw, rb, rg, rbeta = flat_res[5 * r:5 * r + 5]
			rx = ops.as_cl(rx, dt)
			res_x.append(rx)
			if rw is None:
				res_y.append(rx); res_aff.append((None, None, None, None))
			else:
				res_y.append(ops.conv1d(rx, W.packed_weight(rw, dt, _lib.PACK_FWD), Cout, 1, 1, 1, 0, bias = rb))
				res_aff.append(ConvBnActFrozenStatsFunction._affine(cfg['res_bn'][r], rg, rbeta))
		p_drop = cfg['dropout_p']
		seed, offset = _DropoutState.next(y.numel()) if p_drop > 0 else (0, 0)
		skey = _DropoutState.key(dev) if p_drop > 0 else None
		z = ops.bn_act(y, aff[0], aff[1], act, xlen = xl, res = res_y, rscale = [a[0] for a in res_aff], rshift = [a[1] for a in res_aff], dropout_p = p_drop, seed = seed, offset = offset, step_key = skey)
		ctx.cfg, ctx.n_res, ctx.drop = cfg, n_res, (p_drop, seed, offset, skey)
		ctx.params = (weight, bias, gamma, beta) + tuple(flat_res[5 * r + k] for r in range(n_res) for k in range(1, 5))
		ctx.aff, ctx.res_aff = aff, res_aff
		ctx.x_needs_grad = x.requires_grad or ctx.needs_input_grad[1]
		ctx.save_for_backward(x, y, xl, *res_x, *res_y)
		return z

	@staticmethod
	def _coef(scale, C, dev):
		coef = torch.zeros(3 * C, dtype = torch.float32, device = dev)
		coef[:C] = 1.0 if scale is None else scale
		return coef

	@staticmethod
	def backward(ctx, dz):
		cfg, n_res = ctx.cfg, ctx.n_res
		spec, dt, act = cfg['spec'], cfg['compute_dtype'], cfg['act']
		saved = ctx.saved_tensors
		x, y, xl = saved[:3]
		res_x, res_y = list(saved[3:3 + n_res]), list(saved[3 + n_res:3 + 2 * n_res])
		weight, bias, gamma, beta = ctx.params[:4]
		scale, shift, rmean, rinv = ctx.aff
		p_drop, seed, offset, skey = ctx.drop
		B, Cout, Tout = y.shape
		dev = y.device
		dz = ops.as_cl(dz, dt)
		live = lambda p: p is not None and p.requires_grad
		common = dict(xlen = xl, res = res_y, rscale = [a[0] for a in ctx.res_aff], rshift = [a[1] for a in ctx.res_aff], dropout_p = p_drop, seed = seed, offset = offset, step_key = skey)
		dgamma = dbeta = None
		if scale is not None and (live(gamma) or live(beta)):
			sums = torch.empty(2 * Cout, dtype = torch.float64, device = dev)
			scratch = torch.empty(3 * Cout, dtype = torch.float32, device = dev)
			holder = {}
			def reduce(outs, acc):
				holder['g'] = ops.bn_act_bwd_reduce(dz, y, scale, shift, rmean, rinv, act, sums = sums, write_g = True, gamma = gamma, coef = scratch, dgamma = outs[0], dbeta = outs[1], accumulate = acc, **common)
			dgamma, dbeta = _deliver([gamma, beta], reduce)
			g = holder['g']
		else:
			g = ops.bn_act_bwd_reduce(dz, y, scale, shift, None, None, act, write_g = True, **common)
		dy = g if scale is None else ops.bn_act_bwd_apply(g, y, ConvBnActFrozenStatsFunction._coef(scale, Cout, dev), False)
		dw, db = _deliver([weight, bias], lambda outs, acc: ops.conv1d_wgrad(x, dy, Cout, spec.K, spec.stride, spec.dilation, spec.padding, outs[0], dbias = outs[1], accumulate = acc))
		dx = None
		if ctx.x_needs_grad:
			if spec.stride != 1:
				raise _lib.ConvasrHipError('conv1d dgrad with stride > 1 is not implemented (only the prologue conv is strided and its input needs no gradient)')
			dx = _dgrad(x, dy, weight, spec, dt, ctx.producer_link)
		res_grads = []
		for r in range(n_res):
			rw, rb, rg, rbeta = ctx.params[4 + 4 * r:4 + 4 * r + 4]
			need_rx = ctx.needs_input_grad[7 + 5 * r]
			if rw is None:
				res_grads += [g if need_rx else None, None, None, None, None]
				continue
			rscale, rshift, rrm, rri = ctx.res_aff[r]
			drg = drbeta = None
			if rscale is not None and (live(rg) or live(rbeta)):
				rs = torch.empty(2 * Cout, dtype = torch.float64, device = dev)
				ops.bn_act_bwd_reduce(g, g, None, None, None, None, (_lib.ACT_NONE, 0.0, 0.0), res = [res_y[r]], rscale = [None], rshift = [None], rmean = [rrm], rinvstd = [rri], rsums = [rs], write_g = False)
				def put(outs, acc, rs = rs):
					for o, v in ((outs[0], rs[Cout:]), (outs[1], rs[:Cout])):
						if o is not None:
							o.add_(v.float()) if acc else o.copy_(v.float())
				drg, drbeta = _deliver([rg, rbeta], put)
			dry = g if rscale is None else ops.bn_act_bwd_apply(g, res_y[r], ConvBnActFrozenStatsFunction._coef(rscale, Cout, dev), False)
			W.join_prepack(dev)
			drx = ops.conv1d(dry, W.packed_weight(rw, dt, _lib.PACK_DGRAD), res_x[r].shape[1], 1, 1, 1, 0) if need_rx else None
			if rb is not None:
				rb._convasr_grad_is_zero = False
			drw, drb = _deliver([rw, rb], lambda outs, acc, rx = res_x[r], dry = dry: ops.conv1d_wgrad(rx, dry, Cout, 1, 1, 1, 0, outs[0], dbias = outs[1], accumulate = acc))
			res_grads += [drx, drw, drb, drg, drbeta]
		return (None, dx, dw, db, dgamma, dbeta, None, *res_grads)


class LogSoftmaxFunction(torch.autograd.Function):

	@staticmethod
	def forward(ctx, logits):
		lp = ops.log_softmax(ops.as_cl(logits, torch.float32))
		ctx.save_for_backward(lp)
		return lp

	@staticmethod
	def backward(ctx, g):
		lp, = ctx.saved_tensors
		return ops.log_softmax_bwd(g, lp)


class CtcLossFunction(torch.autograd.Function):

	@staticmethod
	def forward(ctx, log_probs, targets, olen, ylen, blank, norm = None):
		lp = ops.as_cl(log_probs, torch.float32)
		need = log_probs.requires_grad
		nll, grad = ops.ctc_loss(lp, targets, olen, ylen, blank, need_grad = need)
		ctx.norm = norm
		if need:
			ctx.save_for_backward(grad)
		if norm is None:
			return nll
		if norm.dtype == torch.int64 and norm.ndim == 1 and norm.device == nll.device:
			return ops.scale_rows(nll, None, norm)
		return nll / norm

	@staticmethod
	def backward(ctx, g):
		grad, = ctx.saved_tensors
		return ops.scale_rows(grad, g, ctx.norm), None, None, None, None, None


def ctc_loss(log_probs, targets, olen, ylen, blank, norm = None):
	return CtcLossFunction.apply(log_probs, targets, olen, ylen, blank, norm)
```

convasr_amd/ops.py:

```python
import math
import os

import ctypes

import torch

from . import _lib
from ._lib import call, ptr, stream_ptr, dtype_code, require_cuda

HALF_DTYPES = (torch.bfloat16, torch.float16)

ACT_CODES = dict(none = _lib.ACT_NONE, relu = _lib.ACT_RELU, hardtanh = _lib.ACT_HARDTANH, leaky_relu = _lib.ACT_LEAKY_RELU)


def act_args(nonlinearity):
	if nonlinearity is None:
		return _lib.ACT_NONE, 0.0, 0.0
	name = nonlinearity[0]
	if name == 'relu':
		return _lib.ACT_RELU, 0.0, 0.0
	if name == 'hardtanh':
		return _lib.ACT_HARDTANH, float(nonlinearity[1]), float(nonlinearity[2])
	if name == 'leaky_relu':
		return _lib.ACT_LEAKY_RELU, float(nonlinearity[1]) if len(nonlinearity) > 1 else 0.01, 0.0
# ... 394 lines not shown
def grouped_conv1d_dgrad(dy, y_act, w, Cin, Tin, groups, stride = 1, pad = 0):
	B, Cout, Tout = dy.shape
	K = w.shape[2]
	assert is_cl(dy) and (y_act is None or (is_cl(y_act) and y_act.dtype == dy.dtype))
	dx = empty_cl(B, Cin, Tin, dy.dtype, dy.device)
	call('convasr_grouped_conv1d_dgrad', ptr(dy), ptr(y_act), ptr(w), w.stride(0), w.stride(1), w.stride(2), ptr(dx), dtype_code(dy.dtype), B, Cin, Cout, Tin, Tout, K, stride, pad, groups, stream_ptr())
	return dx


def grouped_conv1d_wgrad(x, dy, y_act, dw, dbias, groups, stride = 1, pad = 0, accumulate = False):
	B, Cin, Tin = x.shape
	Cout, Tout, K = dy.shape[1], dy.shape[2], dw.shape[2]
	assert is_cl(x) and is_cl(dy) and dw.dtype == torch.float32 and tuple(dw.shape) == (Cout, Cin // groups, K)
	ws = workspace(_lib.load().convasr_grouped_conv1d_wgrad_workspace_bytes(B, Cin, Cout, K, groups), x.device, 'grouped_wgrad')
	call('convasr_grouped_conv1d_wgrad', ptr(x), ptr(dy), ptr(y_act), ptr(dw), dw.stride(0), dw.stride(1), dw.stride(2), ptr(dbias), ptr(ws), dtype_code(x.dtype), B, Cin, Cout, Tin, Tout, K, stride, pad, groups, int(accumulate), stream_ptr())
	return dw



def bn_finalize(stats, n, gamma, beta, running_mean, running_var, momentum, eps, num_batches_tracked = None):
	if isinstance(stats, ConvStats):
		buf, rows, C = stats.buf, stats.rows, stats.C
	else:
		buf, rows, C = stats, 1, stats.numel() // 2
	out = torch.empty(4, C, dtype = torch.float32, device = buf.device)
	o = out.data_ptr()
	call('convasr_bn_finalize', ptr(buf), rows, n, ptr(gamma), ptr(beta), ptr(running_mean), ptr(running_var), float(momentum), float(eps), o, o + 4 * C, o + 8 * C, o + 12 * C, C, ptr(num_batches_tracked), stream_ptr())
	return out


def _float_array(vals):
	return (ctypes.c_float * max(len(vals), 1))(*[float(v) for v in vals])


def bn_finalize_grouped(stats, n, gammas, betas, running_means, running_vars, momenta, epss, num_batches_tracked):
	k, C, rows = len(stats), stats[0].C, stats[0].rows
	assert all(s_.C == C and s_.rows == rows for s_ in stats)
	out = torch.empty(k, 4, C, dtype = torch.float32, device = stats[0].buf.device)
	call('convasr_bn_finalize_grouped', k, _ptr_array([s_.buf for s_ in stats]), rows, n, _ptr_array(gammas), _ptr_array(betas), _ptr_array(running_means), _ptr_array(running_vars),
		_float_array(momenta), _float_array(epss), _ptr_array([out[i] for i in range(k)]), _ptr_array(num_batches_tracked), C, stream_ptr())
	return [out[i] for i in range(k)]


def bn_bwd_finalize_grouped(sums, gammas, means, invstds, n, coefs, dgammas, dbetas, accumulate):
	k, C = len(sums), sums[0].numel() // 2
	call('convasr_bn_bwd_finalize_grouped', k, _ptr_array(sums), _int_array([1] * k), _ptr_array(gammas), _ptr_array(means), _ptr_array(invstds), _ptr_array(coefs), _ptr_array(dgammas), _ptr_array(dbetas),
		_int_array(accumulate), int(n), C, stream_ptr())


def bn_bwd_reduce_many(dz, gate, dropout_p, ys, means, invstds, gammas, coefs, dgammas, dbetas, accumulate):
	B, C, T = dz.shape
	assert is_cl(dz) and dz.dtype in HALF_DTYPES and all(is_cl(y) and y.dtype == dz.dtype and y.shape == dz.shape for y in ys) and gate.dtype == torch.uint8 and gate.numel() * 8 == dz.numel()
	g = empty_cl(B, C, T, dz.dtype, dz.device)
	k = len(ys)
	ws = workspace(_lib.load().convasr_bn_bwd_reduce_many_workspace_bytes(k, B, T, C), dz.device, 'bn_bwd')
	_lib.timed('hbm:bn_act_bwd_reduce_kernel', 0.0, lambda: call('convasr_bn_bwd_reduce_many', ptr(dz), ptr(gate), float(dropout_p), ptr(g), k, _ptr_array(ys), _ptr_array(means), _ptr_array(invstds), _ptr_array(gammas),
		_ptr_array(coefs), _ptr_array(dgammas), _ptr_array(dbetas), _int_array(accumulate), ptr(ws), dtype_code(dz.dtype), B, T, C, stream_ptr()), nbytes = float(B * T * C * dz.element_size() * (2 + k)))
	return g


def bn_bwd_apply_grouped(g, ys, coefs):
	B, C, T = g.shape
	assert is_cl(g) and g.dtype in HALF_DTYPES and all(is_cl(y) and y.dtype == g.dtype and y.shape == g.shape for y in ys)
	dys = [empty_cl(B, C, T, g.dtype, g.device) for _ in ys]
	_lib.timed('hbm:bn_act_bwd_apply_kernel', 0.0, lambda: call('convasr_bn_bwd_apply_grouped', ptr(g), len(ys), _ptr_array(ys), _ptr_array(coefs), _ptr_array(dys), dtype_code(g.dtype), B, T, C, stream_ptr()), nbytes = float(B * T * C * g.element_size() * (1 + 2 * len(ys))))
	return dys


def bn_eval_scale_shift(gamma, beta, running_mean, running_var, eps):
	C = running_mean.numel()
	out = torch.empty(2, C, dtype = torch.float32, device = running_mean.device)
	call('convasr_bn_eval_scale_shift', ptr(gamma), ptr(beta), ptr(running_mean), ptr(running_var), float(eps), ptr(out[0]), ptr(out[1]), C, stream_ptr())
	return out


def _ptr_array(items):
	import ctypes
	arr = (ctypes.c_void_p * max(len(items), 1))()
	for i, t in enumerate(items):
		arr[i] = None if t is None else t.data_ptr()
	return arr


def bn_act(y, scale, shift, act, xlen = None, res = (), rscale = (), rshift = (), dropout_p = 0.0, seed = 0, offset = 0, out = None, gate = None, step_key = None, planes = None):
	B, C, T = y.shape
	assert gate is None or (gate.dtype == torch.uint8 and gate.numel() * 8 == B * C * T and gate.is_contiguous())
	assert is_cl(y) and all(is_cl(r) and r.dtype == y.dtype for r in res)
	if planes is not None:
		assert y.dtype == torch.float32 and planes in HALF_DTYPES and out is None and scale is not None and act[0] != _lib.ACT_LEAKY_RELU
		z3 = empty_cl(B, 3 * C, T, planes, y.device)
		_lib.timed('hbm:bn_act_fwd_kernel', 0.0, lambda: call('convasr_bn_act_fwd_split3', ptr(y), ptr(z3), dtype_code(planes), ptr(scale), ptr(shift), len(res), _ptr_array(res), _ptr_array(rscale) if rscale else None, _ptr_array(rshift) if rshift else None, act[0], act[1], act[2], float(dropout_p), int(seed), int(offset), step_key, ptr(xlen), B, T, C, ptr(gate), stream_ptr()), nbytes = float(B * T * C * (10 + 4 * len(res))))
		return z3
	z = out if out is not None else empty_cl(B, C, T, y.dtype, y.device)
	_lib.timed('hbm:bn_act_fwd_kernel', 0.0, lambda: call('convasr_bn_act_fwd', ptr(y), ptr(z), dtype_code(y.dtype), ptr(scale), ptr(shift), len(res), _ptr_array(res), _ptr_array(rscale) if rscale else None, _ptr_array(rshift) if rshift else None, act[0], act[1], act[2], float(dropout_p), int(seed), int(offset), step_key, ptr(xlen), B, T, C, ptr(gate), stream_ptr()), nbytes = float(B * T * C * y.element_size() * (2 + len(res))))
	return z


_bn_bwd_ws_bytes = {}


def bn_act_bwd_reduce(dz, y, scale, shift, mean, invstd, act, xlen = None, res = (), rscale = (), rshift = (), rmean = (), rinvstd = (), rsums = (), dropout_p = 0.0, seed = 0, offset = 0, sums = None, write_g = True, gamma = None, coef = None, dgamma = None, dbeta = None, accumulate = False, gate = None, step_key = None):
	B, C, T = y.shape
	assert is_cl(y) and is_cl(dz) and dz.dtype == y.dtype and (gate is None or (not write_g and not res))
	g = empty_cl(B, C, T, y.dtype, y.device) if write_g else None
	nb = _bn_bwd_ws_bytes.get((B, T, C))
	if nb is None:
		nb = _bn_bwd_ws_bytes[(B, T, C)] = _lib.load().convasr_bn_bwd_workspace_bytes(B, T, C)
	ws = workspace(nb, y.device, 'bn_bwd')
	_lib.timed('hbm:bn_act_bwd_reduce_kernel', 0.0, lambda: call('convasr_bn_act_bwd_reduce', ptr(dz), ptr(y), ptr(g), dtype_code(y.dtype), ptr(scale), ptr(shift), ptr(mean), ptr(invstd), len(res), _ptr_array(res), _ptr_array(rscale) if rscale else None, _ptr_array(rshift) if rshift else None, _ptr_array(rmean) if rmean else None, _ptr_array(rinvstd) if rinvstd else None, _ptr_array(rsums) if rsums else None, act[0], act[1], act[2], float(dropout_p), int(seed), int(offset), step_key, ptr(xlen), ptr(sums), ptr(ws), ptr(gamma), ptr(coef), ptr(dgamma), ptr(dbeta), int(accumulate), B, T, C, ptr(gate), stream_ptr()), nbytes = float(B * T * C * y.element_size() * (2 + len(res) + (1 if write_g else 0))))
	return g


def bn_act_bwd_apply(dz_or_g, y, coef, from_dz, scale = None, shift = None, act = (_lib.ACT_NONE, 0.0, 0.0), xlen = None, dropout_p = 0.0, seed = 0, offset = 0, out = None, gate = None, step_key = None, planes = None, hi_only = False):
	B, C, T = y.shape
	if planes is not None and hi_only:
		assert y.dtype == torch.float32 and planes in HALF_DTYPES and out is None
		dy16 = empty_cl(B, C, T, planes, y.device)
		_lib.timed('hbm:bn_act_bwd_apply_kernel', 0.0, lambda: call('convasr_bn_act_bwd_apply_to_half', ptr(dz_or_g), ptr(y), ptr(dy16), dtype_code(planes), ptr(coef), int(from_dz), ptr(scale), ptr(shift), act[0], act[1], act[2], float(dropout_p), int(seed), int(offset), step_key, ptr(xlen), B, T, C, ptr(gate), stream_ptr()), nbytes = float(B * T * C * 10))
		return dy16
	if planes is not None:
		assert y.dtype == torch.float32 and planes in HALF_DTYPES and out is None
		dy3 = empty_cl(B, 3 * C, T, planes, y.device)
		_lib.timed('hbm:bn_act_bwd_apply_kernel', 0.0, lambda: call('convasr_bn_act_bwd_apply_split3', ptr(dz_or_g), ptr(y), ptr(dy3), dtype_code(planes), ptr(coef), int(from_dz), ptr(scale), ptr(shift), act[0], act[1], act[2], float(dropout_p), int(seed), int(offset), step_key, ptr(xlen), B, T, C, ptr(gate), stream_ptr()), nbytes = float(B * T * C * 14))
		return dy3
	dy = out if out is not None else empty_cl(B, C, T, y.dtype, y.device)
	_lib.timed('hbm:bn_act_bwd_apply_kernel', 0.0, lambda: call('convasr_bn_act_bwd_apply', ptr(dz_or_g), ptr(y), ptr(dy), dtype_code(y.dtype), ptr(coef), int(from_dz), ptr(scale), ptr(shift), act[0], act[1], act[2], float(dropout_p), int(seed), int(offset), step_key, ptr(xlen), B, T, C, ptr(gate), stream_ptr()), nbytes = float(B * T * C * y.element_size() * 3))
	return dy


def bn_bwd_apply(g, y, gamma, mean, invstd, sums, dgamma = None, dbeta = None, accumulate = False, need_dy = True, inplace = True):
	B, C, T = y.shape
	dy = (g if inplace else empty_cl(B, C, T, y.dtype, y.device)) if need_dy else None
	call('convasr_bn_bwd_apply', ptr(g), ptr(y), ptr(dy), dtype_code(y.dtype), ptr(gamma), ptr(mean), ptr(invstd), ptr(sums), ptr(dgamma), ptr(dbeta), int(accumulate), B, T, C, stream_ptr())
	return dy



def log_softmax(logits):
	B, C, T = logits.shape
	assert is_cl(logits) and logits.dtype == torch.float32
	out = empty_cl(B, C, T, torch.float32, logits.device)
	call('convasr_log_softmax_fwd', ptr(logits), ptr(out), B * T, C, stream_ptr())
	return out


def log_softmax_bwd(grad_lp, log_probs):
	B, C, T = log_probs.shape
	grad_lp = as_cl(grad_lp, torch.float32)
	out = empty_cl(B, C, T, torch.float32, log_probs.device)
	call('convasr_log_softmax_bwd', ptr(grad_lp), ptr(log_probs), ptr(out), B * T, C, stream_ptr())
	return out


def ctc_loss(log_probs, targets, olen, ylen, blank, need_grad = True):
	B, C, T = log_probs.shape
	assert is_cl(log_probs) and log_probs.dtype == torch.float32
	dev = log_probs.device
	targets = targets.to(device = dev, dtype = torch.int64).contiguous()
	if targets.ndim == 1:
		targets = targets.view(B, -1)
	olen = olen.to(device = dev, dtype = torch.int64).contiguous()
	ylen = ylen.to(device = dev, dtype = torch.int64).contiguous()
	S_max = targets.shape[1]
	if not _lib.load().convasr_ctc_loss_supported(B, T, C, S_max):
		return ctc_loss_long(log_probs, targets, olen, ylen, blank, need_grad = need_grad)
	nbytes = _lib.load().convasr_ctc_workspace_bytes(B, T, S_max)
	if nbytes < 0:
		raise _lib.ConvasrHipError(f'ctc_loss: target length {S_max} unsupported')
	ws = workspace(nbytes, dev, 'ctc')
	nll = torch.empty(B, dtype = torch.float32, device = dev)
	grad = empty_cl(B, C, T, torch.float32, dev) if need_grad else None
	call('convasr_ctc_loss', ptr(log_probs), ptr(targets), ptr(olen), ptr(ylen), ptr(nll), ptr(grad), ptr(ws), B, T, C, S_max, blank, stream_ptr())
	return nll, grad


CTC_LONG_WORKSPACE_CAP = 16 << 30


def ctc_loss_long_tiles():
	lib = _lib.load()
	return lib.convasr_ctc_loss_long_states_per_block(), lib.convasr_ctc_loss_long_chunk_frames()


def ctc_loss_long(log_probs, targets, olen, ylen, blank, need_grad = True, chunk_frames = 0, workspace_cap = CTC_LONG_WORKSPACE_CAP):
	require_cuda(log_probs)
	B, C, T = log_probs.shape
	assert is_cl(log_probs) and log_probs.dtype == torch.float32
	dev = log_probs.device
	if _capturing[0] or torch.cuda.is_current_stream_capturing():
		raise _lib.ConvasrHipError(f'ctc_loss_long: B {B}, T {T} is beyond the one-workgroup CTC kernel, and the tiled kernel (hundreds of launches over a workspace allocated per call) cannot be captured into a graph: run this step eagerly')
	targets = targets.to(device = dev, dtype = torch.int64).contiguous()
	if targets.ndim == 1:
		targets = targets.view(B, -1)
	olen = olen.to(device = dev, dtype = torch.int64).contiguous()
	ylen = ylen.to(device = dev, dtype = torch.int64).contiguous()
	S_max = targets.shape[1]
	lib = _lib.load()
	nbytes = lib.convasr_ctc_loss_long_workspace_bytes(B, T, C, S_max)
	if nbytes < 0:
		raise _lib.ConvasrHipError(f'convasr_ctc_loss_long_workspace_bytes failed: {lib.convasr_last_error().decode()}')
	if nbytes > workspace_cap:
		raise _lib.ConvasrHipError(f'ctc_loss_long: {nbytes} bytes of workspace needed for B {B}, T {T}, S_max {S_max}, above the cap of {workspace_cap}')
	nll = torch.empty(B, dtype = torch.float32, device = dev)
	grad = empty_cl(B, C, T, torch.float32, dev) if need_grad else None
	ws = torch.empty(max(nbytes, 16), dtype = torch.uint8, device = dev)
	call('convasr_ctc_loss_long', ptr(log_probs), ptr(targets), ptr(olen), ptr(ylen), ptr(nll), ptr(grad), ptr(ws), nbytes, B, T, C, S_max, int(blank), int(chunk_frames), stream_ptr())
	return nll, grad


def scale_rows(grad, gscale, gdiv = None):
	B = grad.shape[0]
	out = torch.empty_like(grad)
	assert gdiv is None or (gdiv.dtype == torch.int64 and gdiv.ndim == 1 and gdiv.shape[0] == B and gdiv.device == grad.device)
	call('convasr_scale_rows', ptr(grad), None if gscale is None else ptr(gscale.to(torch.float32).contiguous()), ptr(gdiv), 0 if gdiv is None else gdiv.stride(0), ptr(out), B, grad.numel() // B, stream_ptr())
	return out


def loss_head(loss_vec, ylen_col, ent = None, accumulate_iterations = 1, need_grad = True, loss_scaler = None, metric_scale = 1.0):
	require_cuda(loss_vec)
	B = loss_vec.shape[0]
	lv = loss_vec.detach().to(torch.float32).contiguous()
	assert ylen_col.dtype == torch.int64 and ylen_col.ndim == 1 and ylen_col.shape[0] == B and ylen_col.device == lv.device
	out3 = torch.empty(3, dtype = torch.float32, device = lv.device)
	gvec = torch.empty(B, dtype = torch.float32, device = lv.device) if need_grad else None
	skipped = torch.empty(1, dtype = torch.bool, device = lv.device)
	ent = None if ent is None else ent.detach().to(torch.float32).contiguous()
	call('convasr_loss_head', ptr(lv), ptr(ylen_col), ylen_col.stride(0), ptr(ent), B, float(accumulate_iterations), ptr(out3), ptr(gvec), ptr(skipped), ptr(loss_scaler), float(metric_scale), stream_ptr())
	return out3, gvec, skipped


def entropy(log_probs, olen = None, eps = 1e-9):
	B, C, T = log_probs.shape
	lp = as_cl(log_probs, torch.float32)
	ent = torch.empty(B, dtype = torch.float32, device = lp.device)
	ol = None if olen is None else olen.to(device = lp.device, dtype = torch.int64).contiguous()
	call('convasr_entropy', ptr(lp), ptr(ol), ptr(ent), B, T, C, float(eps), stream_ptr())
	return ent


def weighted_mean_entropy(log_probs, olen = None, eps = 1e-9, eps_id = -1):
	B, C, T = log_probs.shape
	lp = as_cl(log_probs, torch.float32)
	out = torch.empty(B, dtype = torch.float32, device = lp.device)
	ol = None if olen is None else olen.to(device = lp.device, dtype = torch.int64).contiguous()
	call('convasr_weighted_mean_entropy', ptr(lp), ptr(ol), ptr(out), B, T, C, int(eps_id) % C, float(eps), stream_ptr())
	return out


def normalize_signal(signal, eps = 1e-5, denom_multiplier = 1.0):
	require_cuda(signal)
	assert signal.ndim == 2
	if signal.numel() == 0:
		return signal
	signal = signal.contiguous() if signal.dtype in (torch.float32, torch.int16) else signal.float().contiguous()
	B, T = signal.shape
	absmax = torch.empty(B, dtype = torch.float32, device = signal.device)
	call('convasr_signal_absmax', ptr(signal), dtype_code(signal.dtype), B, T, ptr(absmax), stream_ptr())
	x = signal if signal.dtype == torch.float32 else signal.float()
	out = torch.empty_like(x)
	scale = ((absmax + eps) * denom_multiplier).reciprocal()
	call('convasr_scale_rows', ptr(x), ptr(scale), None, 0, ptr(out), B, T, stream_ptr())
	return out


def argmax(log_probs):
	B, C, T = log_probs.shape
	lp = as_cl(log_probs, torch.float32)
	idx = torch.empty(B, T, dtype = torch.int64, device = lp.device)
	call('convasr_argmax', ptr(lp), ptr(idx), B * T, C, stream_ptr())
	return idx



def sumsq(flat_grad, out = None, norm_out = None, norm_scale = 1.0, loss_scaler = None):
	out = out if out is not None else torch.empty(1, dtype = torch.float64, device = flat_grad.device)
	ws = workspace(_lib.load().convasr_sumsq_workspace_bytes(), flat_grad.device, 'sumsq')
	call('convasr_sumsq', ptr(flat_grad), flat_grad.numel(), ptr(out), ptr(ws), ptr(norm_out), float(norm_scale), ptr(loss_scaler), stream_ptr())
	return out


def _scaler_pair(scaler):
	if scaler is None:
		return None, None
	s_in, s_out = scaler
	assert s_in.dtype == s_out.dtype == torch.float32 and s_in.numel() == s_out.numel() == _lib.LOSS_SCALER_FLOATS and s_in.data_ptr() != s_out.data_ptr()
	return s_in, s_out


def sgd_step(p, g, buf, n, sumsq_buf, max_norm, lr, momentum, weight_decay, nesterov, first, grad_out = None, loss_gate = None, grad_scale = 1.0, p16 = None, scaler = None, lr_dev = None):
	assert loss_gate is None or (loss_gate.dtype == torch.float32 and loss_gate.numel() == 1)
	assert p16 is None or (p16.dtype in HALF_DTYPES and p16.numel() == n)
	s_in, s_out = _scaler_pair(scaler)
	call('convasr_sgd_step', ptr(p), ptr(g), ptr(buf), ptr(grad_out), n, ptr(sumsq_buf), float(max_norm), float(lr), float(momentum), float(weight_decay), int(nesterov), int(first), ptr(loss_gate), float(grad_scale), ptr(p16), _lib.BF16 if p16 is None else dtype_code(p16.dtype), ptr(s_in), ptr(s_out), ptr(lr_dev), stream_ptr())


def adamw_step(p, g, exp_avg, exp_avg_sq, n, sumsq_buf, max_norm, lr, beta1, beta2, eps, weight_decay, step_in, step_out, loss_gate = None, grad_scale = 1.0, p16 = None, scaler = None, lr_dev = None):
	assert loss_gate is None or (loss_gate.dtype == torch.float32 and loss_gate.numel() == 1)
	assert p16 is None or (p16.dtype in HALF_DTYPES and p16.numel() == n)
	assert step_in.dtype == step_out.dtype == torch.float32 and step_in.data_ptr() != step_out.data_ptr()
	s_in, s_out = _scaler_pair(scaler)
	call('convasr_adamw_step', ptr(p), ptr(g), ptr(exp_avg), ptr(exp_avg_sq), n, ptr(sumsq_buf), float(max_norm), float(lr), float(beta1), float(beta2), float(eps), float(weight_decay), ptr(step_in), ptr(step_out), ptr(loss_gate), float(grad_scale), ptr(p16), _lib.BF16 if p16 is None else dtype_code(p16.dtype), ptr(s_in), ptr(s_out), ptr(lr_dev), stream_ptr())


def conv1d_dgrad_bn_reduce(dy, packed_dgrad, Cin, K, dil, pad, bn_y, bn_scale, bn_shift, bn_mean, bn_invstd, act, dropout_p, seed, offset, xlen, bn_sums, work = None, gate = None, step_key = None):
	import ctypes
	B, Cout, Tdy = dy.shape
	T = conv_out_len(Tdy, K, 1, dil, pad)
	assert is_cl(dy) and dy.dtype in HALF_DTYPES and is_cl(bn_y) and bn_y.dtype == dy.dtype and tuple(bn_y.shape) == (B, Cin, T) and isinstance(bn_sums, ConvStats) and bn_sums.fits(Cin, B, T, dy.device), (dy.shape, bn_y.shape, Cin, T)
	rows = ctypes.c_int(0)
	dx = empty_cl(B, Cin, T, dy.dtype, dy.device)
	rc = [0]
	def run():
		rc[0] = _lib.call_rc('convasr_conv1d_dgrad_bn_reduce', ptr(dy), ptr(packed_dgrad), ptr(dx), dtype_code(dy.dtype), B, Cout, Cin, Tdy, T, K, dil, pad, ptr(bn_y), ptr(bn_scale), ptr(bn_shift), ptr(bn_mean), ptr(bn_invstd), act[0], act[1], act[2], float(dropout_p), int(seed), int(offset), step_key, ptr(xlen), ptr(bn_sums.buf), ctypes.byref(rows), ptr(gate), stream_ptr())
	family = 'conv1d_igemm_v2s_kernel<bf16>+bn_bwd' if Cout % 64 == 0 else 'conv1d_igemm (other variants)'
	flops, nbytes_ = 2.0 * B * T * Cout * Cin * K if work is None else work, float(B * Tdy * Cout * 2 + K * Cout * Cin * 2 + 2 * B * T * Cin * 2)
	symbol = 'v2s16' if family.startswith('conv1d_igemm_v2s') else None
	if family.startswith('conv1d_igemm_v2s') and memory_bound(flops, nbytes_):
		family = 'hbm:conv1d_igemm_v2s_kernel (memory-bound launches: the 38-class decoder)'
	_lib.timed(family, flops, run, nbytes = nbytes_, symbol = symbol)
	bn_sums.rows = rows.value
	return dx if rc[0] == 0 else None


def bn_bwd_finalize(sums, gamma, mean, invstd, n, coef = None, dgamma = None, dbeta = None, accumulate = False):
	buf, rows, C = (sums.buf, sums.rows, sums.C) if isinstance(sums, ConvStats) else (sums, 1, sums.numel() // 2)
	call('convasr_bn_bwd_finalize', ptr(buf), rows, ptr(gamma), ptr(mean), ptr(invstd), ptr(coef), ptr(dgamma), ptr(dbeta), int(accumulate), int(n), C, stream_ptr())
# ... 546 lines not shown
```

include/convasr_hip.h:

```cpp
#ifndef CONVASR_HIP_H
#define CONVASR_HIP_H

#include <stdint.h>

#ifdef __cplusplus
extern "C" {
#endif

#define CONVASR_ABI_VERSION 10

enum { CONVASR_F32 = 0, CONVASR_BF16 = 1, CONVASR_I16 = 2, CONVASR_F16 = 3 };
enum { CONVASR_ACT_NONE = 0, CONVASR_ACT_RELU = 1, CONVASR_ACT_HARDTANH = 2, CONVASR_ACT_LEAKY_RELU = 3 };
enum { CONVASR_OK = 0, CONVASR_EINVAL = -1, CONVASR_ELAUNCH = -2, CONVASR_EUNSUPPORTED = -3 };

int convasr_abi_version(void);
const char* convasr_last_error(void);


int convasr_convert_layout(const void* src, int src_dtype, int64_t src_sb, int64_t src_sc, int64_t src_st,
                           void* dst, int dst_dtype, int64_t dst_sb, int64_t dst_sc, int64_t dst_st,
                           int B, int C, int T, void* stream);


int convasr_signal_absmax(const void* signal, int signal_dtype, int B, int T, float* absmax, void* stream);

int convasr_logmel_fwd(const void* signal, int signal_dtype, const float* absmax, const float* xlen,
                       const float* window, int win_length, const float* mel_weight, const float* mel_bias,
                       float* out, int B, int T, int nfft, int hop, int nmel, float preemphasis, void* stream);


int convasr_instnorm_fwd(const void* x, int x_dtype, int64_t x_sb, int64_t x_sc, int64_t x_st,
                         void* y, int y_dtype, int64_t y_sb, int64_t y_sc, int64_t y_st,
                         const float* xlen, int B, int C, int T, int T_out, float eps, void* stream);

int convasr_instnorm_running_fwd(const void* x, int x_dtype, int64_t x_sb, int64_t x_sc, int64_t x_st,
                                 void* y, int y_dtype, int64_t y_sb, int64_t y_sc, int64_t y_st,
                                 int B, int C, int T, int T_out, float eps, float* running_mean, float* running_var,
                                 int64_t* num_batches_tracked, float momentum, int training, float* stats_workspace, void* stream);


int convasr_output_lengths(const float* xlen, int B, int T, int64_t* out, void* stream);


int convasr_conv_cout_pad(int cout);

#define CONVASR_W_REFERENCE 0
#define CONVASR_W_KMAJOR 1

int convasr_pack_conv_weight(const float* w, void* packed_fwd, void* packed_dgrad, int dtype, int Cout, int Cin, int K, int w_layout, void* stream);

int convasr_conv1d_fwd(const void* x, const void* wp, void* y, int x_dtype, int y_dtype,
                       int B, int Cin, int Cout, int Tin, int Tout, int K, int stride, int dil, int pad,
                       const float* bias, double* stats, const float* scale, const float* shift,
                       int act, float act_lo, float act_hi, const float* xlen, int* stats_rows, void* stream);
int convasr_conv_stats_max_rows(int B, int Tout);

int convasr_conv1d_fwd_splitk_plan(int x_dtype, int B, int Cin, int Cout, int Tout, int K, int64_t* workspace_bytes);
int convasr_conv1d_fwd_splitk(const void* x, const void* wp, void* y, int x_dtype, int y_dtype,
                              int B, int Cin, int Cout, int Tin, int Tout, int K, int dil, int pad,
                              const float* bias, const float* scale, const float* shift, int act, float act_lo, float act_hi,
                              const float* xlen, int splits, void* workspace, void* stream);

int convasr_fold2_geometry(int K, int pad, int* K_folded, int* pad_folded);
int convasr_fold2_pack_weight(const float* w, int w_layout, void* packed_fwd, int dtype, int Cout, int Cin, int K, int pad, void* stream);
int convasr_fold2_unfold_wgrad(const float* dw_folded, float* dw, int dw_layout, int Cout, int Cin, int K, int pad, int accumulate, void* stream);

int convasr_debug_set_conv_v2(int enable);

int64_t convasr_conv1d_wgrad_workspace_bytes(int B, int Cin, int Cout, int Tin, int Tout, int K, int stride, int dil);

int convasr_conv1d_wgrad(const void* x, const void* dy, float* dw, float* dbias, void* workspace, int dtype,
                         int B, int Cin, int Cout, int Tin, int Tout, int K, int stride, int dil, int pad,
                         int accumulate, int dw_layout, void* stream);


int convasr_grouped_conv1d_fwd(const void* x, const float* w, int64_t w_sco, int64_t w_sj, int64_t w_sk, const float* bias, void* y, int dtype,
                               int B, int Cin, int Cout, int Tin, int Tout, int K, int stride, int pad, int groups, int relu, void* stream);
int convasr_grouped_conv1d_dgrad(const void* dy, const void* y_act, const float* w, int64_t w_sco, int64_t w_sj, int64_t w_sk, void* dx, int dtype,
                                 int B, int Cin, int Cout, int Tin, int Tout, int K, int stride, int pad, int groups, void* stream);
int64_t convasr_grouped_conv1d_wgrad_workspace_bytes(int B, int Cin, int Cout, int K, int groups);
int convasr_grouped_conv1d_wgrad(const void* x, const void* dy, const void* y_act, float* dw, int64_t w_sco, int64_t w_sj, int64_t w_sk, float* dbias,
                                 void* workspace, int dtype, int B, int Cin, int Cout, int Tin, int Tout, int K, int stride, int pad, int groups,
                                 int accumulate, void* stream);


int convasr_bn_finalize(const double* stats, int stats_rows, int64_t n, const float* gamma, const float* beta,
                        float* running_mean, float* running_var, float momentum, float eps,
                        float* mean, float* invstd, float* scale, float* shift, int C,
                        int64_t* num_batches_tracked, void* stream);
int convasr_reduce_rows(const double* part, int rows, int width, double* out, void* stream);

int convasr_bn_eval_scale_shift(const float* gamma, const float* beta, const float* running_mean, const float* running_var,
                                float eps, float* scale, float* shift, int C, void* stream);

int convasr_bn_act_fwd(const void* y, void* z, int dtype, const float* scale, const float* shift,
                       int n_res, const void* const* res, const float* const* rscale, const float* const* rshift,
                       int act, float act_lo, float act_hi, float dropout_p, uint64_t seed, uint64_t offset, const uint64_t* step_key,
                       const float* xlen, int B, int T, int C, uint8_t* gate, void* stream);

int64_t convasr_bn_bwd_workspace_bytes(int B, int T, int C);
int convasr_bn_act_bwd_reduce(const void* dz, const void* y, void* g, int dtype, const float* scale, const float* shift,
                              const float* mean, const float* invstd,
                              int n_res, const void* const* res, const float* const* rscale, const float* const* rshift,
                              const float* const* rmean, const float* const* rinvstd, double* const* rsums,
                              int act, float act_lo, float act_hi, float dropout_p, uint64_t seed, uint64_t offset, const uint64_t* step_key,
                              const float* xlen, double* sums, void* workspace, const float* gamma, float* coef, float* dgamma, float* dbeta,
                              int accumulate, int B, int T, int C, const uint8_t* gate, void* stream);

int convasr_bn_act_bwd_apply(const void* dz_or_g, const void* y, void* dy, int dtype, const float* coef, int from_dz,
                             const float* scale, const float* shift, int act, float act_lo, float act_hi, float dropout_p,
                             uint64_t seed, uint64_t offset, const uint64_t* step_key, const float* xlen, int B, int T, int C, const uint8_t* gate, void* stream);

int convasr_bn_bwd_apply(const void* g, const void* y, void* dy, int dtype, const float* gamma, const float* mean,
                         const float* invstd, const double* sums, float* dgamma, float* dbeta, int accumulate,
                         int B, int T, int C, void* stream);


int convasr_log_softmax_fwd(const float* logits, float* log_probs, int64_t rows, int C, void* stream);
int convasr_log_softmax_bwd(const float* grad_lp, const float* log_probs, float* dlogits, int64_t rows, int C, void* stream);

int64_t convasr_ctc_workspace_bytes(int B, int T, int S_max);
int convasr_ctc_loss(const float* log_probs, const int64_t* targets, const int64_t* olen, const int64_t* ylen,
                     float* nll, float* grad, void* workspace, int B, int T, int C, int S_max, int blank, void* stream);
int convasr_ctc_loss_supported(int B, int T, int C, int S_max);

int convasr_ctc_loss_long_states_per_block(void);
int convasr_ctc_loss_long_chunk_frames(void);
int64_t convasr_ctc_loss_long_workspace_bytes(int B, int T, int C, int S_max);
int convasr_ctc_loss_long(const float* log_probs, const int64_t* targets, const int64_t* olen, const int64_t* ylen, float* nll, float* grad,
                          void* workspace, int64_t workspace_bytes, int B, int T, int C, int S_max, int blank, int chunk_frames, void* stream);
int convasr_scale_rows(const float* grad, const float* gscale, const int64_t* gdiv, int64_t gdiv_stride, float* out, int B, int64_t per_b, void* stream);

int convasr_loss_head(const float* loss_vec, const int64_t* ylen, int64_t ylen_stride, const float* entropy, int B, float accumulate_iterations, float* out3,
                      float* grad_loss_vec, unsigned char* skipped, const float* loss_scaler, float metric_scale, void* stream);

#define CONVASR_LOSS_SCALER_FLOATS 8

int convasr_entropy(const float* log_probs, const int64_t* olen, float* ent, int B, int T, int C, float eps, void* stream);
int convasr_weighted_mean_entropy(const float* log_probs, const int64_t* olen, float* out, int B, int T, int C, int eps_id, float eps, void* stream);
int convasr_argmax(const float* log_probs, int64_t* idx, int64_t rows, int C, void* stream);


int64_t convasr_sumsq_workspace_bytes(void);
int convasr_sumsq(const float* g, int64_t n, double* sumsq, void* workspace, float* norm_out, float norm_scale, const float* loss_scaler, void* stream);
int convasr_sgd_step(float* p, const float* g, float* buf, float* grad_out, int64_t n, const double* sumsq, float max_norm,
                     float lr, float momentum, float weight_decay, int nesterov, int first, const float* loss_gate, float grad_scale,
                     void* p16, int p16_dtype, const float* scaler_in, float* scaler_out, const float* lr_dev, void* stream);
int convasr_adamw_step(float* p, const float* g, float* exp_avg, float* exp_avg_sq, int64_t n, const double* sumsq, float max_norm, float lr,
                       float beta1, float beta2, float eps, float weight_decay, const float* step_in, float* step_out, const float* loss_gate,
                       float grad_scale, void* p16, int p16_dtype, const float* scaler_in, float* scaler_out, const float* lr_dev, void* stream);

int convasr_conv1d_dgrad_bn_reduce(const void* dy, const void* packed_dgrad, void* dx, int dtype, int B, int Cout, int Cin, int T_dy, int T_dx, int K,
                                   int dil, int pad, const void* bn_y, const float* bn_scale, const float* bn_shift, const float* bn_mean,
                                   const float* bn_invstd, int bn_act, float bn_act_lo, float bn_act_hi, float dropout_p, uint64_t seed,
                                   uint64_t offset, const uint64_t* step_key, const float* bn_xlen, double* bn_sums, int* bn_rows, const uint8_t* bn_gate, void* stream);
int convasr_bn_bwd_finalize(const double* sums, int sums_rows, const float* gamma, const float* mean, const float* invstd, float* coef,
                            float* dgamma, float* dbeta, int accumulate, int64_t n, int C, void* stream);


int convasr_conv1x1_grouped(int n, const void* const* x, const void* const* w, void* const* y, const float* const* bias, double* const* stats,
                            const int* cin, const int* cout, const int* accumulate, int dtype, int B, int T, int* stats_rows, void* stream);
int64_t convasr_wgrad1x1_grouped_workspace_bytes(int n, const int* cin, const int* cout, int B, int T);
int convasr_wgrad1x1_grouped(int n, const void* const* x, const void* const* dy, float* const* dw, float* const* zero, const int* cin, const int* cout,
                             const int* accumulate, void* workspace, int dtype, int B, int T, void* stream);
int convasr_bn_finalize_grouped(int count, const double* const* stats, int stats_rows, int64_t n, const float* const* gamma, const float* const* beta,
                                float* const* running_mean, float* const* running_var, const float* momentum, const float* eps, float* const* out,
                                int64_t* const* num_batches_tracked, int C, void* stream);
int convasr_bn_bwd_finalize_grouped(int count, const double* const* sums, const int* sums_rows, const float* const* gamma, const float* const* mean,
                                    const float* const* invstd, float* const* coef, float* const* dgamma, float* const* dbeta, const int* accumulate,
                                    int64_t n, int C, void* stream);
int convasr_bn_bwd_apply_grouped(const void* g, int count, const void* const* y, const float* const* coef, void* const* dy, int dtype, int B, int T, int C, void* stream);
int64_t convasr_bn_bwd_reduce_many_workspace_bytes(int count, int B, int T, int C);
int convasr_bn_bwd_reduce_many(const void* dz, const uint8_t* gate, float dropout_p, void* g, int count, const void* const* y, const float* const* mean,
                               const float* const* invstd, const float* const* gamma, float* const* coef, float* const* dgamma, float* const* dbeta,
                               const int* accumulate, void* workspace, int dtype, int B, int T, int C, void* stream);
int convasr_add16(const void* a, const void* b, void* out, int64_t n, int dtype, void* stream);

int convasr_pack_dgrad_item_bytes(void);
int convasr_pack_dgrad_grouped(const void* items, int n_items, int total_blocks, void* stream);

int64_t convasr_colsum_workspace_bytes(int64_t rows, int C);
int convasr_colsum(const void* y, int dtype, int64_t rows, int C, float* out, void* workspace, int accumulate, void* stream);

int convasr_cast_scale(const void* src, int src_dtype, void* dst, int dst_dtype, int64_t n, float scale, void* stream);


int convasr_split3(const float* x, void* out, int dtype, int64_t rows, int C, int order, void* stream);
int convasr_bn_act_fwd_split3(const void* y, void* z3, int plane_dtype, const float* scale, const float* shift,
                              int n_res, const void* const* res, const float* const* rscale, const float* const* rshift,
                              int act, float act_lo, float act_hi, float dropout_p, uint64_t seed, uint64_t offset, const uint64_t* step_key,
                              const float* xlen, int B, int T, int C, uint8_t* gate, void* stream);
int convasr_bn_act_bwd_apply_split3(const void* dz_or_g, const void* y, void* dy3, int plane_dtype, const float* coef, int from_dz,
                                    const float* scale, const float* shift, int act, float act_lo, float act_hi, float dropout_p,
                                    uint64_t seed, uint64_t offset, const uint64_t* step_key, const float* xlen, int B, int T, int C,
                                    const uint8_t* gate, void* stream);
int convasr_pack_conv_weight_split3(const float* w, int w_layout, void* packed_fwd, void* packed_dgrad, int dgrad_planes, int dtype, int Cout, int Cin, int K, void* stream);
int convasr_bn_act_bwd_apply_to_half(const void* dz_or_g, const void* y, void* dy16, int out_dtype, const float* coef, int from_dz,
                                     const float* scale, const float* shift, int act, float act_lo, float act_hi, float dropout_p,
                                     uint64_t seed, uint64_t offset, const uint64_t* step_key, const float* xlen, int B, int T, int C,
                                     const uint8_t* gate, void* stream);
int convasr_conv1d_wgrad_ld_supported(int dtype, int B, int Cin, int Cout, int Tin, int Tout, int K, int dil, int x_ld, int dy_ld);
int convasr_conv1d_wgrad_ld(const void* x, int x_ld, const void* dy, int dy_ld, float* dw, void* workspace, int dtype,
                            int B, int Cin, int Cout, int Tin, int Tout, int K, int dil, int pad, int accumulate, int dw_layout, void* stream);


int convasr_step_begin(uint64_t* state, void* stream);
int convasr_copy(const void* src, void* dst, int64_t nbytes, void* stream);


int convasr_novograd_step(float* p, const float* g, float* mom, const float* ema_in, float* ema_out, double* g2, const int64_t* offsets,
                          int n_seg, int64_t n, const int64_t* items, int n_items, const int64_t* seg_first, double* item_part,
                          float max_norm, float lr, float beta1, float beta2, float eps, float weight_decay, int dampening, int first,
                          const float* loss_gate, float* total_norm, float grad_scale, void* p16, int p16_dtype, const float* scaler_in,
                          float* scaler_out, const float* lr_dev, void* stream);
int64_t convasr_novograd_item_elems(void);

int64_t convasr_ctc_alignment_workspace_bytes(int B, int T, int S_max);
int convasr_ctc_alignment(const float* log_probs, const int64_t* targets, const int64_t* input_lengths, const int64_t* target_lengths,
                          int64_t* alignment, void* workspace, int B, int T, int C, int S_max, int blank, void* stream);

int convasr_ctc_alignment_long_states_per_block(void);
int convasr_ctc_alignment_long_chunk_frames(void);
int64_t convasr_ctc_alignment_long_workspace_bytes(int B, int T, int S_max);
int convasr_ctc_alignment_long(const float* log_probs, const int64_t* targets, const int64_t* input_lengths, const int64_t* target_lengths,
                               int64_t* alignment, void* workspace, int64_t workspace_bytes, int B, int T, int C, int S_max, int blank,
                               int chunk_frames, void* stream);
int convasr_ctc_alignment_long_parts(const float* log_probs, const int64_t* targets, const int64_t* input_lengths, const int64_t* target_lengths,
                                     int64_t* alignment, void* workspace, int64_t workspace_bytes, int B, int T, int C, int S_max, int blank,
                                     int chunk_frames, int parts, void* stream);

int convasr_collate_pad(const void* packed, const int64_t* offsets, const int64_t* lengths, void* out, int elem_bytes, int B, int rows,
                        int64_t Tpad, void* stream);


int64_t convasr_ctc_beam_search_workspace_bytes(int B, int T, int C, int W, int N, int topk);
int convasr_ctc_beam_search(const float* log_probs, const int64_t* lengths, int64_t* tokens, int32_t* offsets, int64_t* out_lengths,
                            float* log_prob, void* workspace, int B, int T, int C, int blank, int W, int N, float cutoff_prob, int topk,
                            void* stream);

int64_t convasr_ctc_beam_search_lm_workspace_bytes(int B, int T, int C, int W, int N, int topk);
int convasr_ctc_beam_search_lm(const float* log_probs, const int64_t* lengths, int64_t* tokens, int32_t* offsets, int64_t* out_lengths,
                               double* log_prob, void* workspace, int B, int T, int C, int blank, int W, int N, float cutoff_prob, int topk,
                               const uint32_t* node_mask, const int32_t* node_child, const int32_t* node_word, int n_nodes,
                               const double* ent_pb, const int32_t* ent_sl, int n_ent, const int32_t* slots, int n_slots,
                               int space, int order, int start_state, double alpha, double beta, void* stream);

int64_t convasr_ctc_beam_search_wide_workspace_bytes(int B, int T, int C, int W, int N, int topk);
int convasr_ctc_beam_search_wide(const float* log_probs, const int64_t* lengths, int64_t* tokens, int32_t* offsets, int64_t* out_lengths,
                                 float* log_prob, void* workspace, int B, int T, int C, int blank, int W, int N, float cutoff_prob, int topk,
                                 void* stream);
int64_t convasr_ctc_beam_search_lm_wide_workspace_bytes(int B, int T, int C, int W, int N, int topk);
int convasr_ctc_beam_search_lm_wide(const float* log_probs, const int64_t* lengths, int64_t* tokens, int32_t* offsets, int64_t* out_lengths,
                                    double* log_prob, void* workspace, int B, int T, int C, int blank, int W, int N, float cutoff_prob, int topk,
                                    const uint32_t* node_mask, const int32_t* node_child, const int32_t* node_word, int n_nodes,
                                    const double* ent_pb, const int32_t* ent_sl, int n_ent, const int32_t* slots, int n_slots,
                                    int space, int order, int start_state, double alpha, double beta, void* stream);


enum { CONVASR_METRIC_CHARS = 0, CONVASR_METRIC_WORDS = 1 };
#define CONVASR_METRIC_MAX_LEN 16383

int convasr_edit_distance(const int64_t* hyp, const int64_t* hyp_lengths, const int64_t* ref, int64_t ref_stride,
                          const int64_t* ref_lengths, int64_t ref_lengths_stride, int32_t* distance, int32_t* ref_units, int B, int K,
                          int Lh, int Lr, int mode, int64_t space, void* stream);

int convasr_ctc_greedy_collapse(const int64_t* path, const int64_t* lengths, int64_t* tokens, int64_t* out_lengths, int B, int T,
                                int eps, int space, int blank_amount_to_space, void* stream);

int convasr_ctc_greedy_segments_chunk_frames(void);
int64_t convasr_ctc_greedy_segments_workspace_bytes(int B, int T);
int convasr_ctc_greedy_segments(const int64_t* path, const int64_t* lengths, int64_t* tokens, int32_t* frames, int64_t* counts,
                                int64_t* seg_first, int32_t* seg_begin, int32_t* seg_end, void* workspace, int64_t workspace_bytes, int B, int T,
                                int eps, int space, int blank_amount_to_space, int split_words, void* stream);


int64_t convasr_nw_align_workspace_bytes(int N, int La, int Lb);
// ... 64 lines not shown
```

Baseline: 58660.

## Fuse CTC gradient, loss scaling, log-softmax backward and head padding into one kernel

CTC loss now keeps its alpha/beta lattices and defers the gradient to backward. A new kernel there computes per-frame posteriors, applies the loss scale and normalisation, runs log-softmax backward, and writes the result straight into the padded half-precision head-conv gradient buffer, with partial bias sums reduced by a second small kernel. This removes the separate fp32 CTC gradient, scale_rows, log_softmax_bwd, layout conversion and bias colsum passes over the output. In exchange it adds token tensors and autograd plumbing with an epoch check that falls back to the dense path. It only applies when C is at most 64 and the head is a padded K=1 conv.

```diff
diff --git a/convasr_amd/_lib.py b/convasr_amd/_lib.py
--- a/convasr_amd/_lib.py
+++ b/convasr_amd/_lib.py
@@ -51,6 +51,10 @@
 	convasr_log_softmax_bwd = (c_int, [c_p, c_p, c_p, c_i64, c_int, c_p]),
 	convasr_ctc_workspace_bytes = (c_i64, [c_int, c_int, c_int]),
 	convasr_ctc_loss = (c_int, [c_p, c_p, c_p, c_p, c_p, c_p, c_p, c_int, c_int, c_int, c_int, c_int, c_p]),
+	convasr_ctc_grad = (c_int, [c_p, c_p, c_p, c_p, c_p, c_p, c_p, c_int, c_int, c_int, c_int, c_int, c_p]),
+	convasr_ctc_head_grad_workspace_bytes = (c_i64, [c_int, c_int, c_int]),
+	convasr_ctc_head_grad = (c_int, [c_p, c_p, c_p, c_p, c_p, c_p, c_p, c_p, c_i64, c_p, c_int, c_int, c_p, c_int, c_int, c_int, c_int, c_int, c_p]),
+	convasr_ctc_head_bias = (c_int, [c_p, c_int, c_int, c_int, c_p, c_int, c_p]),
 	convasr_ctc_loss_supported = (c_int, [c_int, c_int, c_int, c_int]),
 	convasr_ctc_loss_long_states_per_block = (c_int, []),
 	convasr_ctc_loss_long_chunk_frames = (c_int, []),
diff --git a/convasr_amd/csrc/common.h b/convasr_amd/csrc/common.h
--- a/convasr_amd/csrc/common.h
+++ b/convasr_amd/csrc/common.h
@@ -118,6 +118,8 @@
 	return v;
 }
 
+__device__ __forceinline__ float log_softmax_bwd_elem(float g, float p, float sum) { return __builtin_fmaf(-p, sum, g); }
+
 enum { LS_SCALE = 0, LS_UNSKIPPED = 1, LS_OVERFLOW = 2, LS_WINDOW = 3, LS_MIN = 4, LS_MAX = 5, LS_FACTOR = 6, LS_SKIPPED_STEPS = 7 };
 struct LossScale { float scale, inv; bool overflow; };
 __device__ __forceinline__ LossScale loss_scale_read(const float* __restrict__ scaler, double norm_sq) {
diff --git a/convasr_amd/csrc/ctc.hip b/convasr_amd/csrc/ctc.hip
--- a/convasr_amd/csrc/ctc.hip
+++ b/convasr_amd/csrc/ctc.hip
@@ -250,12 +250,44 @@
 	}
 }
 
+struct CtcLattices {
+	const float *alpha, *beta, *offs, *tot;
+	int B, T, cap, split_a, split_b;
+};
+
+__device__ __forceinline__ void ctc_frame_posterior(const CtcLattices& q, const float* __restrict__ row, const int64_t* __restrict__ tg, float* mybins,
+                                                    int b, int t, int Tb, int L, int C, int blank, int lane) {
+	const int NB = q.T / CTC_RENORM + 1;
+	for (int c = lane; c < C; c += 64) mybins[c] = 0.f;
+	__builtin_amdgcn_s_waitcnt(0xc07f);
+	__builtin_amdgcn_wave_barrier();
+	const float* ar = q.alpha + ((int64_t)b * q.T + t) * q.cap;
+	const float* br = q.beta + ((int64_t)b * q.T + t) * q.cap;
+	const float* oa = q.offs + (int64_t)b * 2 * NB + (t >> CTC_RENORM_LOG2);
+	const float* ob = q.offs + ((int64_t)q.B + b) * 2 * NB + ((Tb - 1 - t) >> CTC_RENORM_LOG2);
+	const float ti = q.tot[2 * b], tr = q.tot[2 * b + 1];
+	const float oa0 = oa[0] - ti, oa1 = oa[NB] - ti, ob0 = ob[0], ob1 = ob[NB];
+	const float lpb = row[blank] * CTC_LOG2E;
+	float blank_sum = 0.f;
+	for (int s = lane; s < L; s += 64) {
+		const float shift = ((s >= q.split_a ? oa1 : oa0) + (s >= q.split_b ? ob1 : ob0)) - tr;
+		const float ab = ar[s] + br[s];
+		if (s & 1) {
+			const int c = (int)tg[s >> 1];
+			atomicAdd(mybins + c, __builtin_amdgcn_exp2f(ab + (shift - row[c] * CTC_LOG2E)));
+		} else blank_sum += __builtin_amdgcn_exp2f(ab + (shift - lpb));
+	}
+	blank_sum = wave_sum(blank_sum);
+	if (lane == 0) atomicAdd(mybins + blank, blank_sum);
+	__builtin_amdgcn_s_waitcnt(0xc07f);
+	__builtin_amdgcn_wave_barrier();
+}
+
 __global__ __launch_bounds__(256) void ctc_grad_kernel(const float* __restrict__ lp, const int64_t* __restrict__ targets, const int64_t* __restrict__ olen,
-                                                       const int64_t* __restrict__ ylen, const float* __restrict__ nll, const float* __restrict__ alpha,
-                                                       const float* __restrict__ beta, const float* __restrict__ offs, const float* __restrict__ tot, float* __restrict__ grad,
-                                                       int B, int T, int C, int S_max, int blank, int t_per_block, int cap, int split_a, int split_b) {
+                                                       const int64_t* __restrict__ ylen, const float* __restrict__ nll, const CtcLattices q, float* __restrict__ grad,
+                                                       int C, int S_max, int blank, int t_per_block) {
 	extern __shared__ float bins[];
-	const int NB = T / CTC_RENORM + 1;
+	const int T = q.T;
 	const int b = blockIdx.y, lane = threadIdx.x & 63, wave = threadIdx.x >> 6;
 	const int Tb = (int)olen[b], S = (int)ylen[b], L = 2 * S + 1;
 	const bool feasible = nll[b] < INFINITY;
@@ -269,32 +301,79 @@
 			for (int c = lane; c < C; c += 64) grow[c] = 0.f;
 			continue;
 		}
-		for (int c = lane; c < C; c += 64) mybins[c] = 0.f;
-		__builtin_amdgcn_s_waitcnt(0xc07f);
-		__builtin_amdgcn_wave_barrier();
-		const float* ar = alpha + ((int64_t)b * T + t) * cap;
-		const float* br = beta + ((int64_t)b * T + t) * cap;
-		const float* oa = offs + (int64_t)b * 2 * NB + (t >> CTC_RENORM_LOG2);
-		const float* ob = offs + ((int64_t)B + b) * 2 * NB + ((Tb - 1 - t) >> CTC_RENORM_LOG2);
-		const float ti = tot[2 * b], tr = tot[2 * b + 1];
-		const float oa0 = oa[0] - ti, oa1 = oa[NB] - ti, ob0 = ob[0], ob1 = ob[NB];
-		const float lpb = row[blank] * CTC_LOG2E;
-		float blank_sum = 0.f;
-		for (int s = lane; s < L; s += 64) {
-			const float shift = ((s >= split_a ? oa1 : oa0) + (s >= split_b ? ob1 : ob0)) - tr;
-			const float ab = ar[s] + br[s];
-			if (s & 1) {
-				const int c = (int)tg[s >> 1];
-				atomicAdd(mybins + c, __builtin_amdgcn_exp2f(ab + (shift - row[c] * CTC_LOG2E)));
-			} else blank_sum += __builtin_amdgcn_exp2f(ab + (shift - lpb));
-		}
-		blank_sum = wave_sum(blank_sum);
-		if (lane == 0) atomicAdd(mybins + blank, blank_sum);
-		__builtin_amdgcn_s_waitcnt(0xc07f);
-		__builtin_amdgcn_wave_barrier();
+		ctc_frame_posterior(q, row, tg, mybins, b, t, Tb, L, C, blank, lane);
 		for (int c = lane; c < C; c += 64) grow[c] = __expf(row[c]) - mybins[c];
 		__builtin_amdgcn_wave_barrier();
 	}
+}
+
+#define CTC_HEAD_CHUNK 256
+#define CTC_HEAD_WAVES 8
+template <typename H>
+__global__ __launch_bounds__(64 * CTC_HEAD_WAVES) void ctc_head_grad_kernel(const float* __restrict__ lp, const int64_t* __restrict__ targets, const int64_t* __restrict__ olen,
+                                                                            const int64_t* __restrict__ ylen, const float* __restrict__ nll, const CtcLattices q,
+                                                                            const float* __restrict__ gscale, const int64_t* __restrict__ gdiv, int64_t gdiv_stride,
+                                                                            H* __restrict__ out, int out_ld, float* __restrict__ part, int C, int S_max, int blank) {
+	extern __shared__ float smem[];
+	const int T = q.T;
+	const int lane = threadIdx.x & 63, wave = threadIdx.x >> 6;
+	const int chunk = blockIdx.x >> 2, w = blockIdx.x & 3;
+	const int64_t rows = (int64_t)q.B * T, r0 = (int64_t)chunk * CTC_HEAD_CHUNK, r1 = min(rows, r0 + CTC_HEAD_CHUNK);
+	float* mybins = smem + wave * C;
+	float* vals = smem + CTC_HEAD_WAVES * C;
+	int b = (int)((r0 + w + 4 * wave) / T), t = (int)(r0 + w + 4 * wave - (int64_t)b * T);
+	for (int k = wave; r0 + w + 4 * k < r1; k += CTC_HEAD_WAVES, t += 4 * CTC_HEAD_WAVES) {
+		const int64_t rr = r0 + w + 4 * k;
+		for (; t >= T; t -= T) ++b;
+		const int Tb = (int)olen[b], L = 2 * (int)ylen[b] + 1;
+		const float* row = lp + rr * C;
+		float gc = 0.f;
+		if (t < Tb && nll[b] < INFINITY) {
+			ctc_frame_posterior(q, row, targets + (int64_t)b * S_max, mybins, b, t, Tb, L, C, blank, lane);
+			if (lane < C) gc = __expf(row[lane]) - mybins[lane];
+		}
+		{
+#pragma clang fp contract(off)
+			const float s0 = gscale ? gscale[b] : 1.f;
+			const float s = gdiv ? s0 / (float)gdiv[b * gdiv_stride] : s0;
+			const float g = gc * s;
+			const float sum = wave_sum(lane < C ? 0.f + g : 0.f);
+			if (lane < C) {
+				float dx = log_softmax_bwd_elem(g, expf(row[lane]), sum);
+				asm volatile("" : "+v"(dx));
+				H h;
+				Elem<H>::store(&h, dx);
+				out[rr * out_ld + lane] = h;
+				vals[k * C + lane] = Elem<H>::load(&h);
+			}
+		}
+		__builtin_amdgcn_wave_barrier();
+	}
+	__syncthreads();
+	if (wave == 0 && lane < C) {
+		float a = 0.f;
+#pragma unroll 8
+		for (int k = 0; r0 + w + 4 * k < r1; ++k) a += vals[k * C + lane];
+		part[((int64_t)chunk * 4 + w) * C + lane] = a;
+	}
+}
+
+__global__ __launch_bounds__(1024) void ctc_head_bias_final_kernel(const float* __restrict__ part, int chunks, int C, float* __restrict__ out, int accumulate) {
+	__shared__ double red[16][64];
+	const int c = threadIdx.x & 63, w = threadIdx.x >> 6;
+	double a = 0;
+	if (c < C)
+#pragma unroll 4
+		for (int i = w; i < chunks; i += 16) {
+			const float* p = part + (int64_t)i * 4 * C + c;
+			a += (double)(p[0] + p[C] + p[2 * C] + p[3 * C]);
+		}
+	red[w][c] = a;
+	__syncthreads();
+	if (w != 0 || c >= C) return;
+	double s = 0;
+	for (int i = 0; i < 16; ++i) s += red[i][c];
+	out[c] = accumulate ? out[c] + (float)s : (float)s;
 }
 
 static int ctc_split(int S_max, int* nph, int* npl) {
@@ -306,6 +385,23 @@
 	return 0;
 }
 
+static CtcLattices ctc_lattices(void* workspace, int B, int T, int nph, int npl) {
+	const int NB = T / CTC_RENORM + 1, cap = 128 * (nph + npl);
+	CtcLattices q;
+	float* alpha = (float*)workspace;
+	float* beta = alpha + (int64_t)B * T * cap;
+	float* offs = beta + (int64_t)B * T * cap;
+	q.alpha = alpha; q.beta = beta; q.offs = offs; q.tot = offs + 4 * (int64_t)B * NB;
+	q.B = B; q.T = T; q.cap = cap; q.split_a = 128 * nph; q.split_b = 128 * npl;
+	return q;
+}
+
+static void ctc_launch_grad(const float* log_probs, const int64_t* targets, const int64_t* olen, const int64_t* ylen, const float* nll, const CtcLattices& q, float* grad,
+                            int C, int S_max, int blank, hipStream_t s) {
+	const int t_per_block = 32;
+	hipLaunchKernelGGL(ctc_grad_kernel, dim3((q.T + t_per_block - 1) / t_per_block, q.B), dim3(256), 4 * (size_t)C * sizeof(float), s, log_probs, targets, olen, ylen, nll, q, grad, C, S_max, blank, t_per_block);
+}
+
 extern "C" int64_t convasr_ctc_workspace_bytes(int B, int T, int S_max) {
 	int nph, npl;
 	if (ctc_split(S_max, &nph, &npl) < 0) return -1;
@@ -331,14 +427,9 @@
 	if (ctc_split(S_max, &nph, &npl) < 0) return convasr_fail(CONVASR_EUNSUPPORTED, "ctc_loss: target length %d > 1023", S_max);
 	CONVASR_CHECK_ARG(C <= 8192, "ctc_loss: C %d > 8192", C);
 	hipStream_t s = (hipStream_t)stream;
-	const int NB = T / CTC_RENORM + 1, cap = 128 * (nph + npl);
-	float* alpha = (float*)workspace;
-	float* beta = alpha + (int64_t)B * T * cap;
-	float* offs = beta + (int64_t)B * T * cap;
-	float* tot = offs + 4 * (int64_t)B * NB;
-	const int t_per_block = 32;
-	dim3 ggrid((T + t_per_block - 1) / t_per_block, B);
-	const size_t gsmem = 4 * (size_t)C * sizeof(float);
+	const int cap = 128 * (nph + npl);
+	const CtcLattices q = ctc_lattices(workspace, B, T, nph, npl);
+	float *alpha = (float*)q.alpha, *beta = (float*)q.beta, *offs = (float*)q.offs, *tot = (float*)q.tot;
 	const size_t lds_fixed = ctc_lds_fixed(T, cap), lds_lp = (size_t)T * (C + 1) * sizeof(float);
 	CONVASR_CHECK_ARG(lds_fixed <= 159 * 1024, "ctc_loss: T %d too long for the edge slots", T);
 	const bool in_lds = lds_fixed + lds_lp <= 159 * 1024;
@@ -355,7 +446,45 @@
 	}
 #undef CTC_CASE
 #undef CTC_LAUNCH
-	if (grad) hipLaunchKernelGGL(ctc_grad_kernel, ggrid, dim3(256), gsmem, s, log_probs, targets, olen, ylen, nll, alpha, beta, offs, tot, grad, B, T, C, S_max, blank, t_per_block, cap, 128 * nph, 128 * npl);
+	if (grad) ctc_launch_grad(log_probs, targets, olen, ylen, nll, q, grad, C, S_max, blank, s);
 	CONVASR_CHECK_LAUNCH("ctc_loss");
 	return 0;
 }
+
+extern "C" int convasr_ctc_grad(const float* log_probs, const int64_t* targets, const int64_t* olen, const int64_t* ylen, const float* nll, const void* workspace,
+                                float* grad, int B, int T, int C, int S_max, int blank, void* stream) {
+	CONVASR_CHECK_ARG(log_probs && targets && olen && ylen && nll && workspace && grad && B > 0 && T > 0 && C > 1 && S_max >= 0 && blank >= 0 && blank < C, "ctc_grad: bad arguments");
+	int nph, npl;
+	if (ctc_split(S_max, &nph, &npl) < 0) return convasr_fail(CONVASR_EUNSUPPORTED, "ctc_grad: target length %d > 1023", S_max);
+	ctc_launch_grad(log_probs, targets, olen, ylen, nll, ctc_lattices(const_cast<void*>(workspace), B, T, nph, npl), grad, C, S_max, blank, (hipStream_t)stream);
+	CONVASR_CHECK_LAUNCH("ctc_grad");
+	return 0;
+}
+
+extern "C" int64_t convasr_ctc_head_grad_workspace_bytes(int B, int T, int C) {
+	return ((int64_t)B * T + CTC_HEAD_CHUNK - 1) / CTC_HEAD_CHUNK * 4 * (int64_t)C * (int64_t)sizeof(float);
+}
+
+extern "C" int convasr_ctc_head_grad(const float* log_probs, const int64_t* targets, const int64_t* olen, const int64_t* ylen, const float* nll, const void* workspace,
+                                     const float* gscale, const int64_t* gdiv, int64_t gdiv_stride, void* head_grad, int head_dtype, int head_channels,
+                                     void* bias_partials, int B, int T, int C, int S_max, int blank, void* stream) {
+	CONVASR_CHECK_ARG(log_probs && targets && olen && ylen && nll && workspace && (gscale || gdiv) && head_grad && bias_partials && B > 0 && T > 0 && S_max >= 0 && blank >= 0 && blank < C, "ctc_head_grad: bad arguments");
+	CONVASR_CHECK_ARG(C > 1 && C <= 64 && head_channels >= C && convasr_is_half(head_dtype), "ctc_head_grad: C %d classes (2 .. 64) into %d channels of a 16-bit type", C, head_channels);
+	int nph, npl;
+	if (ctc_split(S_max, &nph, &npl) < 0) return convasr_fail(CONVASR_EUNSUPPORTED, "ctc_head_grad: target length %d > 1023", S_max);
+	const CtcLattices q = ctc_lattices(const_cast<void*>(workspace), B, T, nph, npl);
+	const int64_t chunks = ((int64_t)B * T + CTC_HEAD_CHUNK - 1) / CTC_HEAD_CHUNK;
+	const size_t smem = (size_t)(CTC_HEAD_WAVES + CTC_HEAD_CHUNK / 4) * C * sizeof(float);
+	CONVASR_DISPATCH_HALF(head_dtype, H, hipLaunchKernelGGL((ctc_head_grad_kernel<H>), dim3((unsigned)(4 * chunks)), dim3(64 * CTC_HEAD_WAVES), smem, (hipStream_t)stream, log_probs, targets, olen, ylen, nll, q,
+	                                                        gscale, gdiv, gdiv_stride, (H*)head_grad, head_channels, (float*)bias_partials, C, S_max, blank));
+	CONVASR_CHECK_LAUNCH("ctc_head_grad");
+	return 0;
+}
+
+extern "C" int convasr_ctc_head_bias(const void* bias_partials, int B, int T, int C, float* dbias, int accumulate, void* stream) {
+	CONVASR_CHECK_ARG(bias_partials && dbias && B > 0 && T > 0 && C > 1 && C <= 64, "ctc_head_bias: bad arguments");
+	const int64_t chunks = ((int64_t)B * T + CTC_HEAD_CHUNK - 1) / CTC_HEAD_CHUNK;
+	hipLaunchKernelGGL(ctc_head_bias_final_kernel, dim3(1), dim3(1024), 0, (hipStream_t)stream, (const float*)bias_partials, (int)chunks, C, dbias, accumulate);
+	CONVASR_CHECK_LAUNCH("ctc_head_bias");
+	return 0;
+}
diff --git a/convasr_amd/csrc/misc.hip b/convasr_amd/csrc/misc.hip
--- a/convasr_amd/csrc/misc.hip
+++ b/convasr_amd/csrc/misc.hip
@@ -178,7 +178,7 @@
 	float s = 0.f;
 	for (int c = lane; c < C; c += 64) s += g[row * C + c];
 	s = wave_sum(s);
-	for (int c = lane; c < C; c += 64) dx[row * C + c] = g[row * C + c] - expf(lp[row * C + c]) * s;
+	for (int c = lane; c < C; c += 64) dx[row * C + c] = log_softmax_bwd_elem(g[row * C + c], expf(lp[row * C + c]), s);
 }
 
 extern "C" int convasr_log_softmax_fwd(const float* logits, float* log_probs, int64_t rows, int C, void* stream) {
diff --git a/convasr_amd/functional.py b/convasr_amd/functional.py
--- a/convasr_amd/functional.py
+++ b/convasr_amd/functional.py
@@ -593,19 +593,69 @@
 class _HeadPad:
 	_pad_bufs = {}
 
+	@staticmethod
+	def applies(dt, spec, Cout, Cin):
+		return dt in ops.HALF_DTYPES and spec.K == 1 and spec.stride == 1 and spec.padding == 0 and Cout < W.HEAD_PAD and Cin % 128 == 0 and os.environ.get('CONVASR_NO_HEAD_PAD') != '1'
+
+	@classmethod
+	def buffer(cls, B, Cout, T, dt, dev):
+		key = (B, T, Cout, dt, dev, torch.cuda.current_stream(dev).cuda_stream)
+		out = None if CAPTURING[0] else cls._pad_bufs.get(key)
+		if CAPTURING[0]:
+			out = ops.zeros_cl(B, W.HEAD_PAD, T, dt, dev)
+		elif out is None:
+			if len(cls._pad_bufs) >= 64:
+				cls._pad_bufs.clear()
+			out = cls._pad_bufs[key] = ops.zeros_cl(B, W.HEAD_PAD, T, dt, dev)
+		return out
+
 	@classmethod
 	def pad_grad(cls, dy, dt):
 		B, Cout, T = dy.shape
-		key = (B, T, Cout, dt, dy.device, torch.cuda.current_stream(dy.device).cuda_stream)
-		out = None if CAPTURING[0] else cls._pad_bufs.get(key)
-		if CAPTURING[0]:
-			out = ops.zeros_cl(B, W.HEAD_PAD, T, dt, dy.device)
-		elif out is None:
-			if len(cls._pad_bufs) >= 64:
-				cls._pad_bufs.clear()
-			out = cls._pad_bufs[key] = ops.zeros_cl(B, W.HEAD_PAD, T, dt, dy.device)
+		out = cls.buffer(B, Cout, T, dt, dy.device)
 		_lib.call('convasr_convert_layout', _lib.ptr(dy), _lib.dtype_code(dy.dtype), dy.stride(0), dy.stride(1), dy.stride(2), _lib.ptr(out), _lib.dtype_code(dt), out.stride(0), out.stride(1), out.stride(2), B, Cout, T, _lib.stream_ptr())
 		return out
+
+
+FUSE_HEAD_GRAD = os.environ.get('CONVASR_NO_HEAD_GRAD_FUSION') != '1'
+_HEAD_LINK_ATTR = '_convasr_head_grad_link'
+_zero_words = {}
+
+
+class _HeadGradLink:
+	CLASSES = 38
+
+	def __init__(self, dt):
+		self.dt, self.pending = dt, None
+
+	def take(self):
+		p, self.pending = self.pending, None
+		return p
+
+	@staticmethod
+	def pop(x):
+		d = getattr(x, '__dict__', None)
+		return d.pop(_HEAD_LINK_ATTR, None) if d else None
+
+	@staticmethod
+	def token(like):
+		z = _zero_words.get(like.device)
+		if z is None:
+			z = _zero_words[like.device] = torch.zeros(1, dtype = torch.float32, device = like.device)
+		return z.expand(like.shape)
+
+	@staticmethod
+	def is_token(g, pending):
+		t = pending['token']
+		return g.data_ptr() == t.data_ptr() and g.shape == t.shape and g.stride() == t.stride() and g.dtype == t.dtype
+
+	@staticmethod
+	def unwatched(x):
+		return FUSE_HEAD_GRAD and not x.retains_grad and not getattr(x, '_backward_hooks', None)
+
+	@staticmethod
+	def dense(g, pending):
+		return pending['dense']() if _HeadGradLink.is_token(g, pending) else g + pending['dense']()
 
 
 class ConvBiasFunction(torch.autograd.Function):
@@ -624,6 +674,10 @@
 			y = ops.conv1d(x, W.head_split_weight(weight, ctx.split, 1 if cfg.get('split_hi_bwd') else 3)[0], Cout, 1, 1, 1, 0, out_dtype = cfg.get('out_dtype', torch.float32), bias = bias, work = 2.0 * B * T * Cout * Cin, family = SPLIT_FAMILY)
 		else:
 			y = ops.conv1d(x, W.packed_weight(weight, dt, _lib.PACK_FWD), weight.shape[0], spec.K, spec.stride, spec.dilation, spec.padding, out_dtype = cfg.get('out_dtype', torch.float32), bias = bias)
+		ctx.head_link = None
+		if FUSE_HEAD_GRAD and not CAPTURING[0] and ctx.split is None and _HeadPad.applies(dt, spec, Cout, Cin) and Cout == _HeadGradLink.CLASSES and y.dtype == torch.float32:
+			ctx.head_link = _HeadGradLink(dt)
+			setattr(y, _HEAD_LINK_ATTR, ctx.head_link)
 		ctx.cfg = cfg
 		ctx.params = (weight, bias)
 		ctx.save_for_backward(x)
@@ -636,6 +690,10 @@
 		weight, bias = ctx.params
 		x, = ctx.saved_tensors
 		Cout = weight.shape[0]
+		padded = ctx.split is None and _HeadPad.applies(dt, spec, Cout, x.shape[1])
+		fused = None if ctx.head_link is None else ctx.head_link.take()
+		if fused is not None and not (padded and FUSE_HEAD_GRAD and _HeadGradLink.is_token(dy, fused)):
+			dy, fused = _HeadGradLink.dense(dy, fused), None
 		if ctx.split is not None:
 			Cin = weight.shape[1]
 			B, _, T = dy.shape
@@ -666,16 +724,18 @@
 					ops.colsum(dy, outs[1], accumulate = acc)
 			dw, db = _deliver([weight, bias], wgrad3)
 			return None, dx, dw, db
-		if dt in ops.HALF_DTYPES and spec.K == 1 and spec.stride == 1 and spec.padding == 0 and Cout < W.HEAD_PAD and x.shape[1] % 128 == 0 and os.environ.get('CONVASR_NO_HEAD_PAD') != '1':
-			dyp = _HeadPad.pad_grad(dy, dt)
+		if padded:
+			dyp = fused['dyp'] if fused is not None else _HeadPad.pad_grad(dy, dt)
 			dx = _dgrad(x, dyp, weight, spec, dt, ctx.producer_link, wd = W.head_dgrad_weight(weight, dt)) if ctx.needs_input_grad[1] else None
 
 			def wgrad(outs, acc):
 				dwp = torch.empty(W.HEAD_PAD, x.shape[1], 1, dtype = torch.float32, device = x.device)
-				dbp = torch.empty(W.HEAD_PAD, dtype = torch.float32, device = x.device) if outs[1] is not None else None
+				dbp = torch.empty(W.HEAD_PAD, dtype = torch.float32, device = x.device) if outs[1] is not None and fused is None else None
 				ops.conv1d_wgrad(x, dyp, W.HEAD_PAD, 1, 1, 1, 0, dwp, dbias = dbp)
+				if fused is not None and outs[1] is not None:
+					fused['lattices'].head_bias(fused['part'], outs[1], accumulate = acc)
 				for o, v in ((outs[0], dwp[:Cout]), (outs[1], None if dbp is None else dbp[:Cout].view(Cout, 1, 1))):
-					if o is None:
+					if o is None or v is None:
 						continue
 					if acc:
 						o.add_(v.view(o.shape))
@@ -869,13 +929,26 @@
 
 	@staticmethod
 	def forward(ctx, logits):
-		lp = ops.log_softmax(ops.as_cl(logits, torch.float32))
-		ctx.save_for_backward(lp)
+		link = _HeadGradLink.pop(logits)
+		x = ops.as_cl(logits, torch.float32)
+		lp = ops.log_softmax(x)
+		ctx.head_link = link if x is logits else None
+		if ctx.head_link is not None:
+			setattr(lp, _HEAD_LINK_ATTR, link)
+			ctx.save_for_backward(lp, logits)
+		else:
+			ctx.save_for_backward(lp)
 		return lp
 
 	@staticmethod
 	def backward(ctx, g):
-		lp, = ctx.saved_tensors
+		lp = ctx.saved_tensors[0]
+		fused = None if ctx.head_link is None else ctx.head_link.take()
+		if fused is not None:
+			if _HeadGradLink.is_token(g, fused) and _HeadGradLink.unwatched(ctx.saved_tensors[1]):
+				ctx.head_link.pending = dict(fused, dense = lambda: ops.log_softmax_bwd(fused['dense'](), lp))
+				return fused['token']
+			g = _HeadGradLink.dense(g, fused)
 		return ops.log_softmax_bwd(g, lp)
 
 
@@ -883,11 +956,16 @@
 
 	@staticmethod
 	def forward(ctx, log_probs, targets, olen, ylen, blank, norm = None):
+		link = _HeadGradLink.pop(log_probs)
 		lp = ops.as_cl(log_probs, torch.float32)
 		need = log_probs.requires_grad
-		nll, grad = ops.ctc_loss(lp, targets, olen, ylen, blank, need_grad = need)
+		defer = need and link is not None and lp is log_probs and (norm is None or (norm.dtype == torch.int64 and norm.ndim == 1 and norm.device == lp.device))
+		nll, grad = ops.ctc_loss(lp, targets, olen, ylen, blank, need_grad = need, keep_lattices = defer)
 		ctx.norm = norm
-		if need:
+		ctx.lattices, ctx.head_link = (grad, link) if isinstance(grad, ops.CtcLattices) else (None, None)
+		if ctx.lattices is not None:
+			ctx.save_for_backward(lp)
+		elif need:
 			ctx.save_for_backward(grad)
 		if norm is None:
 			return nll
@@ -897,6 +975,18 @@
 
 	@staticmethod
 	def backward(ctx, g):
+		if ctx.lattices is not None:
+			lp, = ctx.saved_tensors
+			lat, link, norm = ctx.lattices, ctx.head_link, ctx.norm
+			dense = lambda: ops.scale_rows(lat.grad(), g, norm)
+			if _HeadGradLink.unwatched(lp) and g.is_cuda and g.shape == (lp.shape[0], ):
+				dyp = _HeadPad.buffer(lp.shape[0], lp.shape[1], lp.shape[2], link.dt, lp.device)
+				part = lat.head_grad(g.to(torch.float32).contiguous(), norm, dyp)
+				if part is not None:
+					token = _HeadGradLink.token(lp)
+					link.pending = dict(token = token, dyp = dyp, part = part, lattices = lat, dense = dense)
+					return token, None, None, None, None, None
+			return dense(), None, None, None, None, None
 		grad, = ctx.saved_tensors
 		return ops.scale_rows(grad, g, ctx.norm), None, None, None, None, None
 
diff --git a/convasr_amd/ops.py b/convasr_amd/ops.py
--- a/convasr_amd/ops.py
+++ b/convasr_amd/ops.py
@@ -570,7 +570,49 @@
 	return out
 
 
-def ctc_loss(log_probs, targets, olen, ylen, blank, need_grad = True):
+_ctc_epoch = [0]
+
+
+class CtcLattices:
+
+	def __init__(self, log_probs, targets, olen, ylen, blank, nll, ws):
+		self.log_probs, self.targets, self.olen, self.ylen, self.blank, self.nll, self.ws = log_probs, targets, olen, ylen, int(blank), nll, ws
+		self.epoch = _ctc_epoch[0]
+
+	def valid(self):
+		return self.epoch == _ctc_epoch[0] and not _capturing[0]
+
+	def _args(self):
+		B, C, T = self.log_probs.shape
+		return (ptr(self.log_probs), ptr(self.targets), ptr(self.olen), ptr(self.ylen), ptr(self.nll), ptr(self.ws)), (B, T, C, self.targets.shape[1], self.blank)
+
+	def grad(self):
+		if not self.valid():
+			return ctc_loss(self.log_probs, self.targets, self.olen, self.ylen, self.blank, need_grad = True)[1]
+		B, C, T = self.log_probs.shape
+		grad = empty_cl(B, C, T, torch.float32, self.log_probs.device)
+		head, dims = self._args()
+		call('convasr_ctc_grad', *head, ptr(grad), *dims, stream_ptr())
+		return grad
+
+	def head_grad(self, gscale, gdiv, out):
+		B, C, T = self.log_probs.shape
+		if not self.valid() or C > 64 or out.dtype not in HALF_DTYPES or not is_cl(out) or out.shape[0] != B or out.shape[2] != T or out.shape[1] < C:
+			return None
+		assert gscale is None or (gscale.dtype == torch.float32 and gscale.is_contiguous() and gscale.numel() == B and gscale.device == out.device)
+		assert gdiv is None or (gdiv.dtype == torch.int64 and gdiv.ndim == 1 and gdiv.shape[0] == B and gdiv.device == out.device)
+		part = torch.empty(_lib.load().convasr_ctc_head_grad_workspace_bytes(B, T, C) // 4, dtype = torch.float32, device = out.device)
+		head, dims = self._args()
+		call('convasr_ctc_head_grad', *head, ptr(gscale), ptr(gdiv), 0 if gdiv is None else gdiv.stride(0), ptr(out), dtype_code(out.dtype), out.shape[1], ptr(part), *dims, stream_ptr())
+		return part
+
+	def head_bias(self, part, dbias, accumulate = False):
+		B, C, T = self.log_probs.shape
+		assert dbias.dtype == torch.float32 and dbias.is_contiguous() and dbias.numel() == C
+		call('convasr_ctc_head_bias', ptr(part), B, T, C, ptr(dbias), int(accumulate), stream_ptr())
+
+
+def ctc_loss(log_probs, targets, olen, ylen, blank, need_grad = True, keep_lattices = False):
 	B, C, T = log_probs.shape
 	assert is_cl(log_probs) and log_probs.dtype == torch.float32
 	dev = log_probs.device
@@ -587,9 +629,11 @@
 		raise _lib.ConvasrHipError(f'ctc_loss: target length {S_max} unsupported')
 	ws = workspace(nbytes, dev, 'ctc')
 	nll = torch.empty(B, dtype = torch.float32, device = dev)
-	grad = empty_cl(B, C, T, torch.float32, dev) if need_grad else None
+	keep_lattices = keep_lattices and not _capturing[0]
+	grad = empty_cl(B, C, T, torch.float32, dev) if need_grad and not keep_lattices else None
+	_ctc_epoch[0] += 1
 	call('convasr_ctc_loss', ptr(log_probs), ptr(targets), ptr(olen), ptr(ylen), ptr(nll), ptr(grad), ptr(ws), B, T, C, S_max, blank, stream_ptr())
-	return nll, grad
+	return nll, (CtcLattices(log_probs, targets, olen, ylen, blank, nll, ws) if keep_lattices else grad)
 
 
 CTC_LONG_WORKSPACE_CAP = 16 << 30
diff --git a/include/convasr_hip.h b/include/convasr_hip.h
--- a/include/convasr_hip.h
+++ b/include/convasr_hip.h
@@ -122,6 +122,13 @@
 int64_t convasr_ctc_workspace_bytes(int B, int T, int S_max);
 int convasr_ctc_loss(const float* log_probs, const int64_t* targets, const int64_t* olen, const int64_t* ylen,
                      float* nll, float* grad, void* workspace, int B, int T, int C, int S_max, int blank, void* stream);
+int convasr_ctc_grad(const float* log_probs, const int64_t* targets, const int64_t* olen, const int64_t* ylen, const float* nll,
+                     const void* workspace, float* grad, int B, int T, int C, int S_max, int blank, void* stream);
+int64_t convasr_ctc_head_grad_workspace_bytes(int B, int T, int C);
+int convasr_ctc_head_grad(const float* log_probs, const int64_t* targets, const int64_t* olen, const int64_t* ylen, const float* nll,
+                          const void* workspace, const float* gscale, const int64_t* gdiv, int64_t gdiv_stride, void* head_grad,
+                          int head_dtype, int head_channels, void* bias_partials, int B, int T, int C, int S_max, int blank, void* stream);
+int convasr_ctc_head_bias(const void* bias_partials, int B, int T, int C, float* dbias, int accumulate, void* stream);
 int convasr_ctc_loss_supported(int B, int T, int C, int S_max);
 
 int convasr_ctc_loss_long_states_per_block(void);
```

New measurement: 58880 (median of 6 runs). About the same (+0.4%).
